# wangrui2025/GDKVM

Measured on AMD Instinct MI355X. Metric: frames/sec (GDKVM forward + argmax mask), EchoNet 112x112x32 clips, higher is better.
Workload: dtype bf16; 1 GPU; BASELINE.json configs[1]: EchoNet-Dynamic 112x112x32 bf16 inference, batch=16 per GPU; clips_per_gpu=16, frames_per_clip=32, image=112x112, heads=1, key_dim=64, rule=delta_sequential, world_size=1, ranks_seen=1

## Files before the change

gdkvm_amd/csrc/conv3x3_tile.hip:

```cpp
#include <atomic>
#include <type_traits>

#include "gdkvm_common.hpp"

namespace {

constexpr int CT_CK = 64;
constexpr int CT_PIX = 160;
constexpr int CT_SLOTS = CT_PIX / 16;
constexpr int CT_MAXMT = 13;
constexpr int CT_VARIANT_128 = 4, CT_VARIANT_64 = 3;

__device__ const uint4 g_ct_zero16 = {0, 0, 0, 0};

template <int I, int E, class F>
__device__ __forceinline__ void static_for_ct(F&& f)
{
    if constexpr (I < E) {
        f(std::integral_constant<int, I>{});
        static_for_ct<I + 1, E>(f);
    }
}

struct ConvTileArgs {
    const bf16_t* x; const bf16_t* w; const float* bias; const bf16_t* res; bf16_t* y;
    const bf16_t* x2; int C1;
    int N, H, W, C, K;
    int fpt, th, tiles_y, ntiles;
    int bw, bh, band_px, npieces;
    int relu;
    float inv_band, inv_bw, inv_tw, inv_w;
    int perm;
};

__device__ __forceinline__ int ct_div(int n, float inv) { return (int)(((float)n + 0.5f) * inv); }

__host__ __device__ __forceinline__ int ct_channel(int kt, int j, int perm)
{
    return perm ? 32 * (kt >> 1) + 8 * (j >> 2) + 4 * (kt & 1) + (j & 3) : 16 * kt + j;
}

template <int NWN, int NTW, bool PK, int NWV = 8, int MAXMT = CT_MAXMT>
__global__ __launch_bounds__(64 * NWV, (NWV == 4 ? 2 : 1)) void conv3x3_tile_kernel(ConvTileArgs a)
{
    constexpr int MW = NWV / NWN, MTW = (MAXMT + MW - 1) / MW;
    extern __shared__ __attribute__((aligned(16))) unsigned char ct_band[];
    const int tid = threadIdx.x, lane = tid & 63, li = lane & 15, g = lane >> 4;
    const int w = __builtin_amdgcn_readfirstlane(tid >> 6), wn = w % NWN, wm = w / NWN;
    const int H = a.H, W = a.W, C = a.C, K = a.K, BW = a.bw;
    const int band_bytes = a.npieces * 1024, nchunk = C / CT_CK;
    const int tpix = a.fpt * a.th * W;
    const int co0 = blockIdx.y * (16 * NTW * NWN) + 16 * NTW * wn;

    f32x4 bias4[NTW];
#pragma unroll
    for (int nt = 0; nt < NTW; ++nt) {
        const int kt = min(co0 / 16 + nt, K / 16 - 1);
        const float* bp = a.bias + ct_channel(kt, 4 * g, a.perm);
        asm volatile("global_load_dwordx4 %0, %1, off" : "=&v"(bias4[nt]) : "v"(bp) : "memory");
    }

    constexpr int PP = NWV == 8 ? 7 : 8;
    int g_pix[PP], g_meta[PP];
#pragma unroll
    for (int u = 0; u < PP; ++u) {
        const int j = w + NWV * u, d = 64 * j + lane, pix = d / CT_SLOTS, c = d - CT_SLOTS * pix;
        const int f = ct_div(pix, a.inv_band), r = pix - f * (a.bh * BW), by = ct_div(r, a.inv_bw), bx = r - by * BW;
        g_pix[u] = (f * H + by) * W + bx;
        const bool live = j < a.npieces && c < 8 && pix < a.band_px && bx >= 1 && bx <= W;
        g_meta[u] = live ? (by << 16 | (c * 8) << 8 | f) : -1;
    }
    struct Geo { const bf16_t* b1; const bf16_t* b2; int y0, nfr; };
    auto geo_of = [&](int tile) __attribute__((always_inline)) {
        const int ty = tile % a.tiles_y, fg = tile / a.tiles_y;
        Geo q;
        q.y0 = ty * a.th - 1;
        q.nfr = min(a.fpt, a.N - fg * a.fpt);
        const long long px0 = ((long long)fg * a.fpt * H + q.y0) * W - 1;
        q.b1 = a.x + px0 * (a.x2 ? a.C1 : C);
        q.b2 = a.x2 ? a.x2 + px0 * (C - a.C1) - a.C1 : a.x;
        return q;
    };
    auto fetch = [&](const Geo q, int chunk, int buf) __attribute__((always_inline)) {
        const int y0 = q.y0, nfr = q.nfr;
        const bool second = a.x2 != nullptr && chunk * CT_CK >= a.C1;
        const int cs = a.x2 ? (second ? C - a.C1 : a.C1) : C;
        const bf16_t* origin = (second ? q.b2 : q.b1) + chunk * CT_CK;
#pragma unroll
        for (int u = 0; u < PP; ++u) {
            const int j = w + NWV * u;
            const int yy = y0 + (g_meta[u] >> 16);
            const bool ok = g_meta[u] >= 0 && (unsigned)yy < (unsigned)H && (g_meta[u] & 255) < nfr;
            const bf16_t* src = ok ? origin + g_pix[u] * cs + ((g_meta[u] >> 8) & 255) : reinterpret_cast<const bf16_t*>(&g_ct_zero16);
            unsigned char* dst = j < a.npieces ? ct_band + buf * band_bytes + 1024 * j : ct_band + 2 * band_bytes;
            __builtin_amdgcn_global_load_lds(src, reinterpret_cast<__attribute__((address_space(3))) void*>(reinterpret_cast<uintptr_t>(dst)), 16, 0, 0);
        }
    };

    int tile = blockIdx.x;
    Geo cur = geo_of(min(tile, a.ntiles - 1));
    if (tile < a.ntiles) fetch(cur, 0, 0);

    unsigned pbase[MTW];
#pragma unroll
    for (int m = 0; m < MTW; ++m) {
        const int p = min(16 * (wm + MW * m) + li, tpix - 1);
        const int f = ct_div(p, a.inv_tw), r = p - f * (a.th * W), py = ct_div(r, a.inv_w), px = r - py * W;
        pbase[m] = (unsigned)(((f * a.bh + py) * BW + px) * CT_PIX + g * 16);
    }
    const bf16_t* wrow[NTW];
#pragma unroll
    for (int nt = 0; nt < NTW; ++nt) {
        const int kt = min(co0 / 16 + nt, K / 16 - 1);
        if constexpr (PK) wrow[nt] = a.w + (size_t)kt * (9 * C * 16) + lane * 8;
        else wrow[nt] = a.w + (size_t)ct_channel(kt, li, a.perm) * 9 * C + 8 * g;
    }

    const int nks = nchunk * 18;
    static_assert(NTW == 1 || NTW == 2, "wwait names the fragments of one or two output tiles");
    struct WF { bf16x8 f[NTW]; };
    auto wload = [&](WF& o, int ks) __attribute__((always_inline)) {
        ks = ks >= nks ? ks - nks : ks;
        size_t off;
        if constexpr (PK) off = (size_t)ks * 512;
        else {
            const int chunk = ks / 18, r = ks - 18 * chunk, tap = r >> 1, kh = r & 1;
            off = (size_t)tap * C + chunk * CT_CK + 32 * kh;
        }
#pragma unroll
        for (int nt = 0; nt < NTW; ++nt) asm volatile("global_load_dwordx4 %0, %1, off" : "=&v"(o.f[nt]) : "v"(wrow[nt] + off) : "memory");
    };
    auto wwait = [&](WF& o, auto nc) __attribute__((always_inline)) {
        constexpr int N = decltype(nc)::value;
        if constexpr (NTW == 1) asm volatile("s_waitcnt vmcnt(%1)" : "+v"(o.f[0]) : "n"(N) : "memory");
        else asm volatile("s_waitcnt vmcnt(%2)" : "+v"(o.f[0]), "+v"(o.f[1]) : "n"(N) : "memory");
    };
    int gc = 0;
    constexpr int WD = 3, KU = 6;
    WF wr[WD];
#pragma unroll
    for (int j = 0; j < WD; ++j) wload(wr[j], j);
    for (; tile < a.ntiles; tile += gridDim.x) {
        const Geo nxt = geo_of(min(tile + (int)gridDim.x, a.ntiles - 1));
        f32x4 acc[MTW][NTW];
#pragma unroll
        for (int m = 0; m < MTW; ++m)
#pragma unroll
            for (int nt = 0; nt < NTW; ++nt) acc[m][nt] = f32x4{0.f, 0.f, 0.f, 0.f};
        for (int chunk = 0; chunk < nchunk; ++chunk, ++gc) {
            const int buf = gc & 1;
            asm volatile("s_waitcnt vmcnt(%0) lgkmcnt(0)" ::"n"(WD * NTW) : "memory");
            asm volatile("s_barrier" ::: "memory");
            {
                const bool more = chunk + 1 < nchunk;
                Geo q;
                q.b1 = more ? cur.b1 : nxt.b1; q.b2 = more ? cur.b2 : nxt.b2; q.y0 = more ? cur.y0 : nxt.y0; q.nfr = more ? cur.nfr : nxt.nfr;
                fetch(q, more ? chunk + 1 : 0, buf ^ 1);
            }
            const unsigned char* band = ct_band + buf * band_bytes;
            auto load_x = [&](bf16x8 (&xb)[MTW], int r) __attribute__((always_inline)) {
                r = min(r, 17);
                const int tap = r >> 1, kh = r & 1, dy = tap / 3, dx = tap - 3 * dy;
                const unsigned off = (unsigned)((dy * BW + dx) * CT_PIX + kh * 64);
#pragma unroll
                for (int m = 0; m < MTW; ++m) {
                    xb[m] = *reinterpret_cast<const bf16x8*>(band + pbase[m] + off);
                }
            };
            auto mfmas = [&](const bf16x8 (&xb)[MTW], const WF& wfr) __attribute__((always_inline)) {
#pragma unroll
                for (int m = 0; m < MTW; ++m)
#pragma unroll
                    for (int nt = 0; nt < NTW; ++nt) {
                        acc[m][nt] = __builtin_amdgcn_mfma_f32_16x16x32_bf16(wfr.f[nt], xb[m], acc[m][nt], 0, 0, 0);
                    }
            };
            const int ksb = chunk * 18;
            bf16x8 xa[MTW], xb[MTW];
            load_x(xa, 0);
            auto trip = [&](int r0, auto firstc) __attribute__((always_inline)) {
                constexpr bool FIRST = decltype(firstc)::value;
                static_for_ct<0, KU>([&](auto jc) {
                    constexpr int j = decltype(jc)::value;
                    wwait(wr[j % WD], std::integral_constant<int, (WD - 1) * NTW + (FIRST && j < WD ? PP : 0)>{});
                    if constexpr (j % 2 == 0) { load_x(xb, r0 + j + 1); mfmas(xa, wr[j % WD]); }
                    else { load_x(xa, r0 + j + 1); mfmas(xb, wr[j % WD]); }
                    wload(wr[j % WD], ksb + r0 + j + WD);
                    __builtin_amdgcn_sched_barrier(0);
                });
            };
            trip(0, std::true_type{});
#pragma unroll 1
            for (int r0 = KU; r0 < 18; r0 += KU) trip(r0, std::false_type{});
        }
        {
            const int ty = tile % a.tiles_y, fg = tile / a.tiles_y;
            auto bf4 = [](uint2 rr) { return f32x4{__uint_as_float(rr.x << 16), __uint_as_float(rr.x & 0xffff0000u), __uint_as_float(rr.y << 16), __uint_as_float(rr.y & 0xffff0000u)}; };
            auto pk4 = [](const f32x4& v) { return make_uint2((unsigned)f32_to_bf16(v[0]) | ((unsigned)f32_to_bf16(v[1]) << 16), (unsigned)f32_to_bf16(v[2]) | ((unsigned)f32_to_bf16(v[3]) << 16)); };
            const float lo = a.relu ? 0.f : -INFINITY;
            typedef float f32x2 __attribute__((ext_vector_type(2)));
            if (NTW == 2 && a.perm) {
                if (co0 < K) {
                    unsigned o[MTW];
#pragma unroll
                    for (int m = 0; m < MTW; ++m) {
                        const int p = 16 * (wm + MW * m) + li;
                        const int pc = min(p, tpix - 1);
                        const int f = ct_div(pc, a.inv_tw), r = pc - f * (a.th * W), py = ct_div(r, a.inv_w), px = r - py * W;
                        const int n = fg * a.fpt + f, yy = ty * a.th + py;
                        o[m] = p < tpix && n < a.N && yy < H ? (unsigned)(((n * H + yy) * W + px) * K + co0 + 8 * g) : ~0u;
                    }
                    typedef unsigned u32x4 __attribute__((ext_vector_type(4)));
                    bf16_t* const yout = a.y;
                    const bf16_t* const resp = a.res;
                    const unsigned ofallback = (unsigned)(co0 + 8 * g);
                    auto finish = [&](auto resc) __attribute__((always_inline)) {
                        constexpr bool RES = decltype(resc)::value;
                        static_for_ct<0, (MTW + 3) / 4>([&](auto bc) {
                            constexpr int M0 = 4 * decltype(bc)::value, M1 = M0 + 4 < MTW ? M0 + 4 : MTW;
                            u32x4 rr[4] = {};
                            if constexpr (RES) {
#pragma unroll
                                for (int m = M0; m < M1; ++m)
                                {
                                    const bf16_t* const rp = resp + (o[m] != ~0u ? o[m] : ofallback);
                                    asm volatile("global_load_dwordx4 %0, %1, off" : "=&v"(rr[m - M0]) : "v"(rp) : "memory");
                                }
                                asm volatile("s_waitcnt vmcnt(0)" : "+v"(rr[0]), "+v"(rr[1]), "+v"(rr[2]), "+v"(rr[3]) :: "memory");
                            }
#pragma unroll
                            for (int m = M0; m < M1; ++m) {
                                f32x2 v[4];
#pragma unroll
                                for (int q = 0; q < 4; ++q)
                                    v[q] = f32x2{acc[m][q >> 1][2 * (q & 1)], acc[m][q >> 1][2 * (q & 1) + 1]} + f32x2{bias4[q >> 1][2 * (q & 1)], bias4[q >> 1][2 * (q & 1) + 1]};
                                if constexpr (RES) {
#pragma unroll
                                    for (int q = 0; q < 4; ++q) v[q] += f32x2{__uint_as_float(rr[m - M0][q] << 16), __uint_as_float(rr[m - M0][q] & 0xffff0000u)};
                                }
                                u32x4 ow;
#pragma unroll
                                for (int q = 0; q < 4; ++q) {
                                    v[q] = __builtin_elementwise_max(v[q], f32x2{lo, lo});
                                    ow[q] = (unsigned)f32_to_bf16(v[q][0]) | ((unsigned)f32_to_bf16(v[q][1]) << 16);
                                }
                                bf16_t* const yp = yout + o[m];
                                if (o[m] != ~0u) asm volatile("global_store_dwordx4 %0, %1, off\n\ts_nop 1" :: "v"(yp), "v"(ow) : "memory");
                            }
                        });
                    };
                    if (a.res) finish(std::true_type{}); else finish(std::false_type{});
                }
            } else {
#pragma unroll
                for (int m = 0; m < MTW; ++m) {
                    const int p = 16 * (wm + MW * m) + li;
                    if (p >= tpix) continue;
                    const int f = ct_div(p, a.inv_tw), r = p - f * (a.th * W), py = ct_div(r, a.inv_w), px = r - py * W;
                    const int n = fg * a.fpt + f, yy = ty * a.th + py;
                    if (n >= a.N || yy >= H) continue;
                    const size_t opix = (((size_t)n * H + yy) * W + px) * K;
#pragma unroll
                    for (int nt = 0; nt < NTW; ++nt) {
                        if (co0 + 16 * nt >= K) continue;
                        const size_t o = opix + ct_channel(co0 / 16 + nt, 4 * g, a.perm);
                        f32x4 v = acc[m][nt] + bias4[nt];
                        if (a.res) v += bf4(*reinterpret_cast<const uint2*>(a.res + o));
                        v = __builtin_elementwise_max(v, f32x4{lo, lo, lo, lo});
                        *reinterpret_cast<uint2*>(a.y + o) = pk4(v);
                    }
                }
            }
        }
        cur = nxt;
    }
    asm volatile("s_waitcnt vmcnt(0)" ::: "memory");
}

__global__ __launch_bounds__(256) void conv3x3_pack_kernel(const uint4* w, uint4* packed, int K, int C)
{
    const int nks = C / CT_CK * 18;
    const size_t total = (size_t)(K / 16) * nks * 64;
    for (size_t i = (size_t)blockIdx.x * 256 + threadIdx.x; i < total; i += (size_t)gridDim.x * 256) {
        const int lane = (int)(i & 63), li = lane & 15, g = lane >> 4;
        const size_t f = i >> 6;
        const int ks = (int)(f % nks), kt = (int)(f / nks);
        const int chunk = ks / 18, r = ks - 18 * chunk, tap = r >> 1, kh = r & 1;
        packed[i] = w[(((size_t)ct_channel(kt, li, K % 32 == 0) * 9 + tap) * C + chunk * CT_CK + 32 * kh + 8 * g) / 8];
    }
}

__global__ __launch_bounds__(256) void conv3x3_pack_dgrad_kernel(const bf16_t* w, uint4* packed, int K, int C)
{
    const int nks = K / CT_CK * 18;
    const size_t total = (size_t)(C / 16) * nks * 64;
    for (size_t i = (size_t)blockIdx.x * 256 + threadIdx.x; i < total; i += (size_t)gridDim.x * 256) {
        const int lane = (int)(i & 63), li = lane & 15, g = lane >> 4;
        const size_t f = i >> 6;
        const int ks = (int)(f % nks), ct = (int)(f / nks);
        const int chunk = ks / 18, r = ks - 18 * chunk, tap = r >> 1, kh = r & 1;
        const int c = ct_channel(ct, li, C % 32 == 0), ftap = 8 - tap;
        const bf16_t* src = w + ((size_t)(chunk * CT_CK + 32 * kh + 8 * g) * 9 + ftap) * C + c;
        unsigned short e[8];
#pragma unroll
        for (int j = 0; j < 8; ++j) e[j] = src[(size_t)j * 9 * C];
        packed[i] = make_uint4(e[0] | (unsigned)e[1] << 16, e[2] | (unsigned)e[3] << 16, e[4] | (unsigned)e[5] << 16, e[6] | (unsigned)e[7] << 16);
    }
}

}

struct PackTrainLayer { const float* w; uint4* fwd; uint4* dgrad; int K, C; long long sK, sC, sR, sS; };
struct PackTrainArgs { PackTrainLayer l[GDKVM_PACK_MAX_LAYERS]; };

namespace {
__global__ __launch_bounds__(256) void conv3x3_pack_train_kernel(PackTrainArgs a)
{
    const PackTrainLayer L = a.l[blockIdx.y];
    if (!L.w) return;
    const int K = L.K, C = L.C;
    const size_t nf = (size_t)(K / 16) * (C / CT_CK * 18) * 64, nd = (size_t)(C / 16) * (K / CT_CK * 18) * 64;
    auto bf = [](float x) { return (unsigned)f32_to_bf16(x); };
    for (size_t i = (size_t)blockIdx.x * 256 + threadIdx.x; i < nf + nd; i += (size_t)gridDim.x * 256) {
        const bool fwd = i < nf;
        const size_t ii = fwd ? i : i - nf;
        const int lane = (int)(ii & 63), li = lane & 15, g = lane >> 4;
        const size_t f = ii >> 6;
        float e[8];
        if (fwd) {
            const int nks = C / CT_CK * 18, ks = (int)(f % nks), kt = (int)(f / nks);
            const int chunk = ks / 18, r = ks - 18 * chunk, tap = r >> 1, kh = r & 1;
            const float* src = L.w + (long long)ct_channel(kt, li, K % 32 == 0) * L.sK + (long long)(tap / 3) * L.sR + (long long)(tap % 3) * L.sS
                               + (long long)(chunk * CT_CK + 32 * kh + 8 * g) * L.sC;
#pragma unroll
            for (int j = 0; j < 8; ++j) e[j] = src[(long long)j * L.sC];
        } else {
            const int nks = K / CT_CK * 18, ks = (int)(f % nks), ct = (int)(f / nks);
            const int chunk = ks / 18, r = ks - 18 * chunk, tap = r >> 1, kh = r & 1, ftap = 8 - tap;
            const float* src = L.w + (long long)ct_channel(ct, li, C % 32 == 0) * L.sC + (long long)(ftap / 3) * L.sR + (long long)(ftap % 3) * L.sS
                               + (long long)(chunk * CT_CK + 32 * kh + 8 * g) * L.sK;
#pragma unroll
            for (int j = 0; j < 8; ++j) e[j] = src[(long long)j * L.sK];
        }
        const uint4 o = make_uint4(bf(e[0]) | bf(e[1]) << 16, bf(e[2]) | bf(e[3]) << 16, bf(e[4]) | bf(e[5]) << 16, bf(e[6]) | bf(e[7]) << 16);
        (fwd ? L.fwd : L.dgrad)[ii] = o;
    }
}
}

extern "C" int gdkvm_conv3x3_pack_weights_train(int nlayers, const void* const* w, void* const* packed_fwd, void* const* packed_dgrad,
                                                const int* K, const int* C, const long long* strides, void* stream)
{
    if (nlayers < 0 || nlayers > GDKVM_PACK_MAX_LAYERS) return gdkvm_fail(GDKVM_ERR_SHAPE, "conv3x3_pack_weights_train: %d layers (at most %d per call)", nlayers, GDKVM_PACK_MAX_LAYERS);
    if (nlayers == 0) return GDKVM_OK;
    if (!w || !packed_fwd || !packed_dgrad || !K || !C || !strides) return gdkvm_fail(GDKVM_ERR_ARG, "conv3x3_pack_weights_train: null pointer");
    PackTrainArgs a{};
    for (int i = 0; i < nlayers; ++i) {
        if (K[i] <= 0 || C[i] <= 0 || K[i] % CT_CK || C[i] % CT_CK)
            return gdkvm_fail(GDKVM_ERR_SHAPE, "conv3x3_pack_weights_train: layer %d K=%d C=%d (multiples of 64)", i, K[i], C[i]);
        if (!w[i] || !packed_fwd[i] || !packed_dgrad[i] || !gdkvm_aligned16(packed_fwd[i]) || !gdkvm_aligned16(packed_dgrad[i]))
            return gdkvm_fail(GDKVM_ERR_ARG, "conv3x3_pack_weights_train: layer %d: null or unaligned pointer", i);
        a.l[i] = PackTrainLayer{static_cast<const float*>(w[i]), static_cast<uint4*>(packed_fwd[i]), static_cast<uint4*>(packed_dgrad[i]), K[i], C[i],
                                strides[4 * i], strides[4 * i + 1], strides[4 * i + 2], strides[4 * i + 3]};
    }
    if (int rc = gdkvm_check_device()) return rc;
    hipLaunchKernelGGL(conv3x3_pack_train_kernel, dim3(48, (unsigned)nlayers), dim3(256), 0, static_cast<hipStream_t>(stream), a);
    GDKVM_LAUNCH_CHECK("conv3x3_pack_train_kernel");
    return GDKVM_OK;
}

extern "C" int gdkvm_conv3x3_pack_weights_dgrad(const void* w, void* packed, int K, int C, int io_dtype, void* stream)
{
    if (io_dtype != GDKVM_BF16) return gdkvm_fail(GDKVM_ERR_DTYPE, "conv3x3_pack_weights_dgrad: only bf16 is implemented");
    if (K <= 0 || C <= 0 || K % CT_CK || C % 16) return gdkvm_fail(GDKVM_ERR_SHAPE, "conv3x3_pack_weights_dgrad: K=%d C=%d (K a multiple of 64, C of 16)", K, C);
    if (!w || !packed || !gdkvm_aligned16(w) || !gdkvm_aligned16(packed)) return gdkvm_fail(GDKVM_ERR_ARG, "conv3x3_pack_weights_dgrad: null or unaligned pointer");
    if (int rc = gdkvm_check_device()) return rc;
    const size_t total = (size_t)(C / 16) * (K / CT_CK * 18) * 64;
    hipLaunchKernelGGL(conv3x3_pack_dgrad_kernel, dim3((unsigned)((total + 255) / 256)), dim3(256), 0, static_cast<hipStream_t>(stream),
                       static_cast<const bf16_t*>(w), static_cast<uint4*>(packed), K, C);
    GDKVM_LAUNCH_CHECK("conv3x3_pack_dgrad_kernel");
    return GDKVM_OK;
}

extern "C" int gdkvm_conv3x3_pack_weights(const void* w, void* packed, int K, int C, int io_dtype, void* stream)
{
    if (io_dtype != GDKVM_BF16) return gdkvm_fail(GDKVM_ERR_DTYPE, "conv3x3_pack_weights: only bf16 is implemented");
    if (K <= 0 || C <= 0 || K % 16 || C % CT_CK) return gdkvm_fail(GDKVM_ERR_SHAPE, "conv3x3_pack_weights: K=%d C=%d (K a multiple of 16, C of 64)", K, C);
    if (!w || !packed || !gdkvm_aligned16(w) || !gdkvm_aligned16(packed)) return gdkvm_fail(GDKVM_ERR_ARG, "conv3x3_pack_weights: null or unaligned pointer");
    if (int rc = gdkvm_check_device()) return rc;
    const size_t total = (size_t)(K / 16) * (C / CT_CK * 18) * 64;
    hipLaunchKernelGGL(conv3x3_pack_kernel, dim3((unsigned)((total + 255) / 256)), dim3(256), 0, static_cast<hipStream_t>(stream),
                       static_cast<const uint4*>(w), static_cast<uint4*>(packed), K, C);
    GDKVM_LAUNCH_CHECK("conv3x3_pack_kernel");
    return GDKVM_OK;
}

namespace {
template <int NWN, int NTW, int NWV = 8, int MAXMT = CT_MAXMT>
void launch_tile(bool packed, dim3 grid, size_t lds, hipStream_t st, const ConvTileArgs& a)
{
    if (packed) hipLaunchKernelGGL((conv3x3_tile_kernel<NWN, NTW, true, NWV, MAXMT>), grid, dim3(64 * NWV), lds, st, a);
    else hipLaunchKernelGGL((conv3x3_tile_kernel<NWN, NTW, false, NWV, MAXMT>), grid, dim3(64 * NWV), lds, st, a);
}
template <int NWN, int NTW, int NWV = 8, int MAXMT = CT_MAXMT>
bool setattr_tile()
{
    return hipFuncSetAttribute(reinterpret_cast<const void*>(conv3x3_tile_kernel<NWN, NTW, true, NWV, MAXMT>), hipFuncAttributeMaxDynamicSharedMemorySize, 113 * 1024) == hipSuccess
        && hipFuncSetAttribute(reinterpret_cast<const void*>(conv3x3_tile_kernel<NWN, NTW, false, NWV, MAXMT>), hipFuncAttributeMaxDynamicSharedMemorySize, 113 * 1024) == hipSuccess;
}
}

int gdkvm_conv3x3_tile_launch(const void* x, const void* x2, int C1, const void* w, const float* bias, const void* residual, void* y,
                              int N, int C, int H, int W, int K, int relu, int variant, int packed, hipStream_t st)
{
    if (variant == 0 && K % 128 == 0 && CT_VARIANT_128 == 4) {
        if (gdkvm_conv3x3_tile_launch(x, x2, C1, w, bias, residual, y, N, C, H, W, K, relu, 4, packed, st) == 0) return 0;
        variant = 2;
    }
    if (variant == 0 && K % 128 != 0 && (H * W <= 16 * 7 || 2 * W <= 16 * 7)) {
        if (gdkvm_conv3x3_tile_launch(x, x2, C1, w, bias, residual, y, N, C, H, W, K, relu, 5, packed, st) == 0) return 0;
        variant = 3;
    }
    if (C % CT_CK || K % 16 || W > 64 || W < 1 || H < 1 || N < 1 || variant < 0 || variant > 5) return 1;
    if (variant == 4 && K % 128) return 1;
    const bool half = variant == 4 || variant == 5;
    if (x2 && (C1 <= 0 || C1 >= C || C1 % CT_CK)) return 1;
    ConvTileArgs a;
    a.x2 = static_cast<const bf16_t*>(x2); a.C1 = x2 ? C1 : C;
    a.x = static_cast<const bf16_t*>(x); a.w = static_cast<const bf16_t*>(w); a.bias = bias;
    a.res = static_cast<const bf16_t*>(residual); a.y = static_cast<bf16_t*>(y);
    a.N = N; a.H = H; a.W = W; a.C = C; a.K = K; a.relu = relu;
    const int maxpix = half ? 16 * 7 : 16 * CT_MAXMT;
    const int maxpieces = half ? 32 : 56;
    if (H * W <= maxpix) { a.th = H; a.fpt = maxpix / (H * W); a.tiles_y = 1; if (a.fpt > N) a.fpt = N; }
    else { a.fpt = 1; a.th = maxpix / W; if (a.th < 1) return 1; a.tiles_y = (H + a.th - 1) / a.th; }
    a.bw = W + 2; a.bh = a.th + 2;
    auto pieces = [&]() { a.band_px = a.fpt * a.bh * a.bw; return (a.band_px * CT_SLOTS + 63) / 64; };
    while (pieces() > maxpieces && a.fpt > 1) --a.fpt;
    while (pieces() > maxpieces && a.th > 1) { --a.th; a.bh = a.th + 2; a.tiles_y = (H + a.th - 1) / a.th; }
    a.npieces = pieces();
    if (a.npieces > maxpieces) return 1;
    a.inv_band = 1.0f / (float)(a.bh * a.bw); a.inv_bw = 1.0f / (float)a.bw;
    a.inv_tw = 1.0f / (float)(a.th * W); a.inv_w = 1.0f / (float)W;
    a.perm = K % 32 == 0;
    const long long groups = (N + a.fpt - 1) / a.fpt;
    const long long ntiles = groups * a.tiles_y;
    if (ntiles <= 0 || ntiles > 0x7fffffffLL) return 1;
    a.ntiles = (int)ntiles;
    if (variant == 0) variant = K % 128 == 0 ? 2 : CT_VARIANT_64;
    const int kwg = (variant == 2 || variant == 4) ? 128 : 64;
    const int gy = (K + kwg - 1) / kwg;
    const size_t lds = (size_t)2 * a.npieces * 1024 + 1024;
    int per = (half ? 512 : 256) / gy; if (per < 1) per = 1;
    const int gx = (int)(ntiles < per ? ntiles : per);
    static std::atomic<unsigned long long> done_mask{0};
    int dev = 0;
    if (hipGetDevice(&dev) != hipSuccess) return 1;
    const unsigned long long bit = 1ull << (dev & 63);
    if (!(done_mask.load(std::memory_order_relaxed) & bit)) {
        if (!setattr_tile<4, 1>() || !setattr_tile<4, 2>() || !setattr_tile<2, 2>() || !setattr_tile<4, 2, 4, 7>() || !setattr_tile<2, 2, 4, 7>()) return 1;
        done_mask.fetch_or(bit, std::memory_order_relaxed);
    }
    switch (variant) {
        case 1: launch_tile<4, 1>(packed, dim3(gx, gy), lds, st, a); break;
        case 2: launch_tile<4, 2>(packed, dim3(gx, gy), lds, st, a); break;
        case 4: launch_tile<4, 2, 4, 7>(packed, dim3(gx, gy), lds, st, a); break;
        case 5: launch_tile<2, 2, 4, 7>(packed, dim3(gx, gy), lds, st, a); break;
        default: launch_tile<2, 2>(packed, dim3(gx, gy), lds, st, a); break;
    }
    return 0;
}
```

gdkvm_amd/csrc/conv_dispatch.hip:

```cpp
#include "gdkvm_common.hpp"

int gdkvm_conv3x3_c64_launch(const void* x, const void* w, const float* bias, const void* residual, void* y, int N, int H, int W,
                             int relu, int packed, hipStream_t st);
int gdkvm_conv3x3_tile_launch(const void* x, const void* x2, int C1, const void* w, const float* bias, const void* residual, void* y,
                              int N, int C, int H, int W, int K, int relu, int variant, int packed, hipStream_t st);
int gdkvm_conv_igemm_launch(const void* x, const void* wpacked, const float* bias, const void* residual, void* y,
                            int N, int C, int H, int W, int K, int R, int S, int stride, int pad, int relu,
                            const void* w2packed, const float* bias2, void* y2, hipStream_t st);

extern "C" int gdkvm_conv_bias_act(const void* x, const void* w, const float* bias, const void* residual, void* y,
                                   int N, int C, int H, int W, int K, int R, int S, int stride, int pad, int relu, int kernel,
                                   int io_dtype, void* stream)
{
    if (io_dtype != GDKVM_BF16) return gdkvm_fail(GDKVM_ERR_DTYPE, "conv_bias_act: only bf16 is implemented");
    if (N < 0 || C <= 0 || H <= 0 || W <= 0 || K <= 0 || R <= 0 || S <= 0 || stride <= 0 || pad < 0 || C % 8 || K % 8
        || H + 2 * pad < R || W + 2 * pad < S)
        return gdkvm_fail(GDKVM_ERR_SHAPE, "conv_bias_act: N=%d C=%d H=%d W=%d K=%d %dx%d stride %d pad %d (C, K multiples of 8)",
                          N, C, H, W, K, R, S, stride, pad);
    const bool packed = kernel & GDKVM_CONV_PACKED_WEIGHTS;
    kernel &= ~GDKVM_CONV_PACKED_WEIGHTS;
    if (kernel != 0 && (kernel < 4 || kernel > 11)) return gdkvm_fail(GDKVM_ERR_ARG, "conv_bias_act: kernel=%d (0 = by shape, 4, 5, 6..8, 9, 10, 11)", kernel);
    if (kernel == 9) {
        if (!packed) return gdkvm_fail(GDKVM_ERR_ARG, "conv_bias_act: kernel 9 reads the gdkvm_conv_igemm_pack_weights copy of the weights (flag %d)", GDKVM_CONV_PACKED_WEIGHTS);
        if (C % 32 || K % 128) return gdkvm_fail(GDKVM_ERR_SHAPE, "conv_bias_act: kernel 9 needs C a multiple of 32 and K of 128 (C=%d K=%d)", C, K);
        if (N == 0) return GDKVM_OK;
        if (!x || !w || !bias || !y) return gdkvm_fail(GDKVM_ERR_ARG, "conv_bias_act: null pointer");
        if (!gdkvm_aligned16(x) || !gdkvm_aligned16(w) || !gdkvm_aligned16(y) || !gdkvm_aligned16(bias) || (residual && !gdkvm_aligned16(residual)))
            return gdkvm_fail(GDKVM_ERR_ARG, "conv_bias_act: pointers must be 16-byte aligned");
        if (int rc = gdkvm_check_device()) return rc;
        if (gdkvm_conv_igemm_launch(x, w, bias, residual, y, N, C, H, W, K, R, S, stride, pad, relu, nullptr, nullptr, nullptr, static_cast<hipStream_t>(stream)))
            return gdkvm_fail(GDKVM_ERR_SHAPE, "conv_bias_act: N=%d C=%d H=%d W=%d K=%d %dx%d stride %d pad %d is too large for 32-bit offsets", N, C, H, W, K, R, S, stride, pad);
        GDKVM_LAUNCH_CHECK("conv_igemm_kernel");
        return GDKVM_OK;
    }
    if (packed && (C % 64 || K % 16))
        return gdkvm_fail(GDKVM_ERR_ARG, "conv_bias_act: packed weights need C a multiple of 64 and K of 16 (C=%d K=%d)", C, K);
    if (!(R == 3 && S == 3 && stride == 1 && pad == 1))
        return gdkvm_fail(GDKVM_ERR_SHAPE, "conv_bias_act: %dx%d stride %d pad %d is not served by the 3x3 / 1 / 1 kernels: kernel 9 (the "
                                           "implicit-GEMM kernel, packed weights) or the framework convolution + gdkvm_bias_act", R, S, stride, pad);
    if (N == 0) return GDKVM_OK;
    if (!x || !w || !bias || !y) return gdkvm_fail(GDKVM_ERR_ARG, "conv_bias_act: null pointer");
    if (!gdkvm_aligned16(x) || !gdkvm_aligned16(w) || !gdkvm_aligned16(y) || !gdkvm_aligned16(bias) || (residual && !gdkvm_aligned16(residual)))
        return gdkvm_fail(GDKVM_ERR_ARG, "conv_bias_act: pointers must be 16-byte aligned");
    if ((size_t)N * H * W * C >= (1ull << 31) || (size_t)N * H * W * K >= (1ull << 31))
        return gdkvm_fail(GDKVM_ERR_SHAPE, "conv_bias_act: tensor too large for 32-bit offsets");
    if (int rc = gdkvm_check_device()) return rc;
    hipStream_t st = static_cast<hipStream_t>(stream);
    const bool c64 = C == 64 && K == 64;
    if (kernel == 4 && !c64) return gdkvm_fail(GDKVM_ERR_SHAPE, "conv_bias_act: kernel 4 serves 64 -> 64 channels only (C=%d K=%d)", C, K);
    if (kernel == 4 || (kernel == 0 && c64)) {
        if (gdkvm_conv3x3_c64_launch(x, w, bias, residual, y, N, H, W, relu, packed ? 1 : 0, st)) return gdkvm_fail(GDKVM_ERR_SHAPE, "conv_bias_act: too many tiles");
        GDKVM_LAUNCH_CHECK("conv3x3_c64_kernel");
        return GDKVM_OK;
    }
    if (gdkvm_conv3x3_tile_launch(x, nullptr, 0, w, bias, residual, y, N, C, H, W, K, relu, kernel >= 10 ? kernel - 6 : (kernel >= 6 ? kernel - 5 : 0), packed ? 1 : 0, st))
        return gdkvm_fail(GDKVM_ERR_SHAPE, "conv_bias_act: C=%d K=%d %dx%d is not served by the hand-written kernels (C a multiple of 64, K of "
                                           "16, rows of at most 64 pixels): use the framework convolution + gdkvm_bias_act", C, K, H, W);
    GDKVM_LAUNCH_CHECK("conv3x3_tile_kernel");
    return GDKVM_OK;
}

extern "C" int gdkvm_conv_cat_bias_act(const void* x1, const void* x2, const void* w, const float* bias, const void* residual, void* y,
                                       int N, int C1, int C2, int H, int W, int K, int relu, int kernel, int io_dtype, void* stream)
{
    if (io_dtype != GDKVM_BF16) return gdkvm_fail(GDKVM_ERR_DTYPE, "conv_cat_bias_act: only bf16 is implemented");
    const bool packed = kernel & GDKVM_CONV_PACKED_WEIGHTS;
    kernel &= ~GDKVM_CONV_PACKED_WEIGHTS;
    if (kernel != 0 && (kernel < 5 || kernel > 11 || kernel == 9)) return gdkvm_fail(GDKVM_ERR_ARG, "conv_cat_bias_act: kernel=%d (0, 5..8, 10, 11)", kernel);
    if (N < 0 || C1 <= 0 || C2 <= 0 || C1 % 64 || C2 % 64 || H <= 0 || W <= 0 || K <= 0 || K % 16)
        return gdkvm_fail(GDKVM_ERR_SHAPE, "conv_cat_bias_act: N=%d C1=%d C2=%d H=%d W=%d K=%d (C1, C2 multiples of 64, K of 16)", N, C1, C2, H, W, K);
    if (N == 0) return GDKVM_OK;
    if (!x1 || !x2 || !w || !bias || !y) return gdkvm_fail(GDKVM_ERR_ARG, "conv_cat_bias_act: null pointer");
    if (!gdkvm_aligned16(x1) || !gdkvm_aligned16(x2) || !gdkvm_aligned16(w) || !gdkvm_aligned16(y) || !gdkvm_aligned16(bias) || (residual && !gdkvm_aligned16(residual)))
        return gdkvm_fail(GDKVM_ERR_ARG, "conv_cat_bias_act: pointers must be 16-byte aligned");
    if ((size_t)N * H * W * (C1 + C2) >= (1ull << 31) || (size_t)N * H * W * K >= (1ull << 31))
        return gdkvm_fail(GDKVM_ERR_SHAPE, "conv_cat_bias_act: tensor too large for 32-bit offsets");
    if (int rc = gdkvm_check_device()) return rc;
    if (gdkvm_conv3x3_tile_launch(x1, x2, C1, w, bias, residual, y, N, C1 + C2, H, W, K, relu, kernel >= 10 ? kernel - 6 : (kernel >= 6 ? kernel - 5 : 0), packed ? 1 : 0,
                                  static_cast<hipStream_t>(stream)))
        return gdkvm_fail(GDKVM_ERR_SHAPE, "conv_cat_bias_act: %dx%d is not served (rows of at most 64 pixels)", H, W);
    GDKVM_LAUNCH_CHECK("conv3x3_tile_kernel");
    return GDKVM_OK;
}

extern "C" int gdkvm_conv_down_bias_act(const void* x, const void* w, const float* bias, void* y, int relu,
                                        const void* w_down, const float* bias_down, void* y_down,
                                        int N, int C, int H, int W, int K, int R, int S, int stride, int pad, int io_dtype, void* stream)
{
    if (io_dtype != GDKVM_BF16) return gdkvm_fail(GDKVM_ERR_DTYPE, "conv_down_bias_act: only bf16 is implemented");
    if (N < 0 || C <= 0 || H <= 0 || W <= 0 || K <= 0 || R <= 0 || S != R || !(R & 1) || stride <= 0 || pad != R / 2 || C % 32 || K % 128)
        return gdkvm_fail(GDKVM_ERR_SHAPE, "conv_down_bias_act: N=%d C=%d H=%d W=%d K=%d %dx%d stride %d pad %d (odd square window, pad = R/2, "
                                           "C a multiple of 32, K of 128)", N, C, H, W, K, R, S, stride, pad);
    if (N == 0) return GDKVM_OK;
    if (!x || !w || !bias || !y || !w_down || !y_down) return gdkvm_fail(GDKVM_ERR_ARG, "conv_down_bias_act: null pointer");
    const void* ptrs[] = {x, w, bias, y, w_down, y_down};
    for (const void* p : ptrs) if (!gdkvm_aligned16(p)) return gdkvm_fail(GDKVM_ERR_ARG, "conv_down_bias_act: pointers must be 16-byte aligned");
    if (bias_down && !gdkvm_aligned16(bias_down)) return gdkvm_fail(GDKVM_ERR_ARG, "conv_down_bias_act: pointers must be 16-byte aligned");
    if (int rc = gdkvm_check_device()) return rc;
    if (gdkvm_conv_igemm_launch(x, w, bias, nullptr, y, N, C, H, W, K, R, S, stride, pad, relu, w_down, bias_down, y_down, static_cast<hipStream_t>(stream)))
        return gdkvm_fail(GDKVM_ERR_SHAPE, "conv_down_bias_act: tensor too large for 32-bit offsets");
    GDKVM_LAUNCH_CHECK("conv_igemm_kernel");
    return GDKVM_OK;
}
```

gdkvm_amd/csrc/epilogue.hip:

```cpp
#include <type_traits>

#include <stdlib.h>
#include "gdkvm_common.hpp"

namespace {

template <int IO, bool FIXED>
__global__ __launch_bounds__(256) void bias_act_kernel(const void* x, const float* bias, const void* res, void* y,
                                                       size_t nvec, int C, int relu)
{
    constexpr int V = IO == GDKVM_F32 ? 4 : 8;
    constexpr int UNR = 4;
    typedef uint4 vec_t;
    const vec_t* xv = static_cast<const vec_t*>(x);
    const vec_t* rv = static_cast<const vec_t*>(res);
    vec_t* yv = static_cast<vec_t*>(y);
    const size_t stride = (size_t)gridDim.x * 256;
    float bfix[V];
    if constexpr (FIXED) {
        const int c0 = (int)((((size_t)blockIdx.x * 256 + threadIdx.x) * V) % (size_t)C);
#pragma unroll
        for (int j = 0; j < V; j += 4) {
            const f32x4 b4 = *reinterpret_cast<const f32x4*>(bias + c0 + j);
            bfix[j] = b4[0]; bfix[j + 1] = b4[1]; bfix[j + 2] = b4[2]; bfix[j + 3] = b4[3];
// ... 71 lines not shown
        uint4 win[9];
#pragma unroll
        for (int dy = 0; dy < 3; ++dy)
#pragma unroll
            for (int dx = 0; dx < 3; ++dx) {
                const int ih = 2 * oh - 1 + dy, iw = 2 * ow - 1 + dx;
                const bool ok = ih >= 0 && ih < H && iw >= 0 && iw < W;
                const int hh = ok ? ih : 2 * oh, ww = ok ? iw : 2 * ow;
                win[3 * dy + dx] = xv[(((size_t)n * Hp + hh) * Wp + ww) * cg + c];
            }
        float m[V];
#pragma unroll
        for (int j = 0; j < V; ++j) m[j] = -INFINITY;
#pragma unroll
        for (int t = 0; t < 9; ++t) {
            const unsigned w4[4] = {win[t].x, win[t].y, win[t].z, win[t].w};
#pragma unroll
            for (int j = 0; j < 4; ++j) {
                if constexpr (IO == GDKVM_F32) m[j] = fmaxf(m[j], __uint_as_float(w4[j]));
                else {
                    m[2 * j] = fmaxf(m[2 * j], __uint_as_float(w4[j] << 16));
                    m[2 * j + 1] = fmaxf(m[2 * j + 1], __uint_as_float(w4[j] & 0xffff0000u));
                }
            }
        }
#pragma unroll
        for (int j = 0; j < V; j += 4) {
            const f32x4 b4 = *reinterpret_cast<const f32x4*>(bias + c * V + j);
#pragma unroll
            for (int q = 0; q < 4; ++q) m[j + q] = fmaxf(m[j + q] + b4[q], 0.f);
        }
        uint4 o;
        if constexpr (IO == GDKVM_F32) {
            o.x = __float_as_uint(m[0]); o.y = __float_as_uint(m[1]); o.z = __float_as_uint(m[2]); o.w = __float_as_uint(m[3]);
        } else {
            o.x = (unsigned)f32_to_bf16(m[0]) | ((unsigned)f32_to_bf16(m[1]) << 16);
            o.y = (unsigned)f32_to_bf16(m[2]) | ((unsigned)f32_to_bf16(m[3]) << 16);
            o.z = (unsigned)f32_to_bf16(m[4]) | ((unsigned)f32_to_bf16(m[5]) << 16);
            o.w = (unsigned)f32_to_bf16(m[6]) | ((unsigned)f32_to_bf16(m[7]) << 16);
        }
        yv[i] = o;
    }
}

template <int IO>
__global__ __launch_bounds__(256) void stem_s2d_kernel(const void* x, void* out, int N, int C, int H, int W, int Cp)
{
    typedef typename std::conditional<IO == GDKVM_F32, float, bf16_t>::type T;
    const T* xi = static_cast<const T*>(x);
    T* o = static_cast<T*>(out);
    const int Ho = H / 2, Wo = W / 2;
    const size_t total = (size_t)N * Ho * Wo;
    for (size_t i = (size_t)blockIdx.x * 256 + threadIdx.x; i < total; i += (size_t)gridDim.x * 256) {
        const int j = (int)(i % Wo);
        const size_t r = i / Wo;
        const int ih = (int)(r % Ho), n = (int)(r / Ho);
        T* dst = o + i * Cp;
        if constexpr (IO == GDKVM_BF16) {
            if (Cp == 16 && C <= 4) {
                unsigned pr[8] = {0, 0, 0, 0, 0, 0, 0, 0};
                for (int c = 0; c < C; ++c) {
                    const bf16_t* src = xi + (((size_t)n * C + c) * H + 2 * ih) * W + 2 * j;
                    pr[2 * c] = *reinterpret_cast<const unsigned*>(src);
                    pr[2 * c + 1] = *reinterpret_cast<const unsigned*>(src + W);
                }
                reinterpret_cast<uint4*>(dst)[0] = make_uint4(pr[0], pr[1], pr[2], pr[3]);
                reinterpret_cast<uint4*>(dst)[1] = make_uint4(pr[4], pr[5], pr[6], pr[7]);
                continue;
            }
        }
        for (int c = 0; c < C; ++c) {
            const T* src = xi + (((size_t)n * C + c) * H + 2 * ih) * W + 2 * j;
            dst[4 * c + 0] = src[0]; dst[4 * c + 1] = src[1]; dst[4 * c + 2] = src[W]; dst[4 * c + 3] = src[W + 1];
        }
        for (int c = 4 * C; c < Cp; ++c) dst[c] = T(0);
    }
}

}

extern "C" int gdkvm_bias_act(const void* x, const float* bias, const void* residual, void* y,
                              size_t rows, int C, int relu, int io_dtype, void* stream)
{
    if (C <= 0) return gdkvm_fail(GDKVM_ERR_SHAPE, "bias_act: C=%d", C);
    if (io_dtype != GDKVM_F32 && io_dtype != GDKVM_BF16) return gdkvm_fail(GDKVM_ERR_DTYPE, "bias_act: io_dtype=%d", io_dtype);
    const int V = io_dtype == GDKVM_F32 ? 4 : 8;
    if (C % V) return gdkvm_fail(GDKVM_ERR_SHAPE, "bias_act: C=%d must be a multiple of %d", C, V);
    if (rows == 0) return GDKVM_OK;
    if (!x || !bias || !y) return gdkvm_fail(GDKVM_ERR_ARG, "bias_act: null pointer");
    if (!gdkvm_aligned16(x) || !gdkvm_aligned16(y) || !gdkvm_aligned16(bias) || (residual && !gdkvm_aligned16(residual)))
        return gdkvm_fail(GDKVM_ERR_ARG, "bias_act: pointers must be 16-byte aligned");
    if (int rc = gdkvm_check_device()) return rc;
    const size_t nvec = rows * (size_t)C / V;
    size_t blocks = (nvec + 255) / 256;
    if (blocks > 256 * 8) blocks = 256 * 8;
    hipStream_t st = static_cast<hipStream_t>(stream);
    const bool fixed = (blocks * 256) % (size_t)(C / V) == 0;
#define GDKVM_BA(IO, FX) hipLaunchKernelGGL((bias_act_kernel<IO, FX>), dim3((unsigned)blocks), dim3(256), 0, st, x, bias, residual, y, nvec, C, relu)
    if (io_dtype == GDKVM_F32) { if (fixed) GDKVM_BA(GDKVM_F32, true); else GDKVM_BA(GDKVM_F32, false); }
    else { if (fixed) GDKVM_BA(GDKVM_BF16, true); else GDKVM_BA(GDKVM_BF16, false); }
#undef GDKVM_BA
    GDKVM_LAUNCH_CHECK("bias_act_kernel");
    return GDKVM_OK;
}

namespace {

__device__ __forceinline__ void unpack8(const uint4& a, float (&v)[8])
{
    const unsigned w[4] = {a.x, a.y, a.z, a.w};
#pragma unroll
    for (int j = 0; j < 4; ++j) { v[2 * j] = __uint_as_float(w[j] << 16); v[2 * j + 1] = __uint_as_float(w[j] & 0xffff0000u); }
}

__global__ __launch_bounds__(256) void upsample_cat_bf16_kernel(const bf16_t* lo, const bf16_t* skip, bf16_t* out,
                                                                int Nimg, int hl, int wl, int H, int W, int C1, int C2,
                                                                float sy, float sx, float inv_c1n, float inv_c2n, float inv_h)
{
    auto qdiv = [](int n, float inv) { return (int)(((float)n + 0.5f) * inv); };
    const int C = C1 + C2, c1n = C1 / 8, c2n = C2 / 8, n1 = W * c1n, n2 = W * c2n, tid = threadIdx.x;
    constexpr int MAXV = 2;
    const bool exact2x = H == 2 * hl && W == 2 * wl;
    for (int row = blockIdx.x; row < Nimg * H; row += gridDim.x) {
        const int n = qdiv(row, inv_h), y = row - n * H;
        const float fy = fmaxf(sy * ((float)y + 0.5f) - 0.5f, 0.f);
        const int y0 = (int)fy, y1 = min(y0 + 1, hl - 1);
        const float ly = fy - (float)y0, hy = 1.f - ly;
        const bf16_t* lo0 = lo + ((size_t)n * hl + y0) * wl * C1;
        const bf16_t* lo1 = lo + ((size_t)n * hl + y1) * wl * C1;
        const bf16_t* sk = skip + (size_t)row * W * C2;
        bf16_t* orow = out + (size_t)row * W * C;
        uint4 cp[MAXV];
#pragma unroll
        for (int u = 0; u < MAXV; ++u) cp[u] = n2 ? *reinterpret_cast<const uint4*>(sk + min(u * 256 + tid, n2 - 1) * 8) : make_uint4(0u, 0u, 0u, 0u);
        if (exact2x) {
            const int nu = (wl + 1) * c1n;
            for (int u0 = 0; u0 < nu; u0 += 256) {
                const int u = min(u0 + tid, nu - 1);
                const int jq = qdiv(u, inv_c1n), c = (u - jq * c1n) * 8, jp = jq - 1;
                const int x0 = max(jp, 0), x1 = min(jp + 1, wl - 1);
                const uint4 t00 = *reinterpret_cast<const uint4*>(lo0 + x0 * C1 + c), t01 = *reinterpret_cast<const uint4*>(lo0 + x1 * C1 + c);
                const uint4 t10 = *reinterpret_cast<const uint4*>(lo1 + x0 * C1 + c), t11 = *reinterpret_cast<const uint4*>(lo1 + x1 * C1 + c);
                if (u0 + tid >= nu) continue;
                float a[8], b[8], cc[8], d[8];
                unpack8(t00, a); unpack8(t01, b); unpack8(t10, cc); unpack8(t11, d);
#pragma unroll
                for (int e = 0; e < 2; ++e) {
                    const int x = 2 * jp + 1 + e;
                    if (x < 0 || x >= W) continue;
                    const float lx = e ? 0.75f : 0.25f, hx = 1.f - lx;
                    unsigned r[4];
#pragma unroll
                    for (int q = 0; q < 4; ++q) {
                        const float v0 = hy * (hx * a[2 * q] + lx * b[2 * q]) + ly * (hx * cc[2 * q] + lx * d[2 * q]);
                        const float v1 = hy * (hx * a[2 * q + 1] + lx * b[2 * q + 1]) + ly * (hx * cc[2 * q + 1] + lx * d[2 * q + 1]);
                        r[q] = (unsigned)f32_to_bf16(v0) | ((unsigned)f32_to_bf16(v1) << 16);
                    }
                    *reinterpret_cast<uint4*>(orow + x * C + c) = make_uint4(r[0], r[1], r[2], r[3]);
                }
            }
        } else
        for (int j0 = 0; j0 < n1; j0 += MAXV * 256) {
            uint4 t[MAXV][4];
            float lx[MAXV];
            int oidx[MAXV];
#pragma unroll
            for (int u = 0; u < MAXV; ++u) {
                const int j = min(j0 + u * 256 + tid, n1 - 1);
                const int x = qdiv(j, inv_c1n), c = (j - x * c1n) * 8;
                const float fx = fmaxf(sx * ((float)x + 0.5f) - 0.5f, 0.f);
                const int x0 = (int)fx, x1 = min(x0 + 1, wl - 1);
                lx[u] = fx - (float)x0;
                oidx[u] = x * C + c;
                t[u][0] = *reinterpret_cast<const uint4*>(lo0 + x0 * C1 + c);
                t[u][1] = *reinterpret_cast<const uint4*>(lo0 + x1 * C1 + c);
                t[u][2] = *reinterpret_cast<const uint4*>(lo1 + x0 * C1 + c);
                t[u][3] = *reinterpret_cast<const uint4*>(lo1 + x1 * C1 + c);
            }
#pragma unroll
            for (int u = 0; u < MAXV; ++u) {
                if (j0 + u * 256 + tid >= n1) continue;
                const float hx = 1.f - lx[u];
                float a[8], b[8], cc[8], d[8];
                unpack8(t[u][0], a); unpack8(t[u][1], b); unpack8(t[u][2], cc); unpack8(t[u][3], d);
                unsigned r[4];
#pragma unroll
                for (int q = 0; q < 4; ++q) {
                    const float v0 = hy * (hx * a[2 * q] + lx[u] * b[2 * q]) + ly * (hx * cc[2 * q] + lx[u] * d[2 * q]);
                    const float v1 = hy * (hx * a[2 * q + 1] + lx[u] * b[2 * q + 1]) + ly * (hx * cc[2 * q + 1] + lx[u] * d[2 * q + 1]);
                    r[q] = (unsigned)f32_to_bf16(v0) | ((unsigned)f32_to_bf16(v1) << 16);
                }
                *reinterpret_cast<uint4*>(orow + oidx[u]) = make_uint4(r[0], r[1], r[2], r[3]);
            }
        }
#pragma unroll
        for (int u = 0; u < MAXV; ++u) {
            const int jc = u * 256 + tid;
            if (jc < n2) {
                const int x = qdiv(jc, inv_c2n);
                *reinterpret_cast<uint4*>(orow + x * C + C1 + (jc - x * c2n) * 8) = cp[u];
            }
        }
        for (int jc = MAXV * 256 + tid; jc < n2; jc += 256) {
            const int x = qdiv(jc, inv_c2n);
            *reinterpret_cast<uint4*>(orow + x * C + C1 + (jc - x * c2n) * 8) = *reinterpret_cast<const uint4*>(sk + jc * 8);
        }
    }
}

__global__ __launch_bounds__(256) void upsample_cat_bf16_2x_kernel(const bf16_t* lo, const bf16_t* skip, bf16_t* out,
                                                                   int Nimg, int hl, int wl, int C1, int C2, float inv_c1n, float inv_c2n, float inv_hp)
{
    auto qdiv = [](int n, float inv) { return (int)(((float)n + 0.5f) * inv); };
    const int H = 2 * hl, W = 2 * wl, C = C1 + C2, c1n = C1 / 8, c2n = C2 / 8, n2 = W * c2n, tid = threadIdx.x;
    const int nu = (wl + 1) * c1n, hp = hl + 1;
    for (int rp = blockIdx.x; rp < Nimg * hp; rp += gridDim.x) {
        const int n = qdiv(rp, inv_hp), ip = rp - n * hp - 1;
        const int r0 = max(ip, 0), r1 = min(ip + 1, hl - 1);
        const bf16_t* lo0 = lo + ((size_t)n * hl + r0) * wl * C1;
        const bf16_t* lo1 = lo + ((size_t)n * hl + r1) * wl * C1;
        constexpr int MAXV = 2;
        uint4 cp[2][MAXV];
#pragma unroll
        for (int ey = 0; ey < 2; ++ey) {
            const int y = min(max(2 * ip + 1 + ey, 0), H - 1);
            const bf16_t* sk = skip + ((size_t)n * H + y) * W * C2;
#pragma unroll
            for (int u = 0; u < MAXV; ++u) cp[ey][u] = n2 ? *reinterpret_cast<const uint4*>(sk + min(u * 256 + tid, n2 - 1) * 8) : make_uint4(0u, 0u, 0u, 0u);
        }
        for (int u0 = 0; u0 < nu; u0 += 256) {
            const int u = min(u0 + tid, nu - 1);
            const int jq = qdiv(u, inv_c1n), c = (u - jq * c1n) * 8, jp = jq - 1;
            const int x0 = max(jp, 0), x1 = min(jp + 1, wl - 1);
            const uint4 t00 = *reinterpret_cast<const uint4*>(lo0 + x0 * C1 + c), t01 = *reinterpret_cast<const uint4*>(lo0 + x1 * C1 + c);
            const uint4 t10 = *reinterpret_cast<const uint4*>(lo1 + x0 * C1 + c), t11 = *reinterpret_cast<const uint4*>(lo1 + x1 * C1 + c);
            if (u0 + tid >= nu) continue;
            float a[8], b[8], cc[8], d[8];
            unpack8(t00, a); unpack8(t01, b); unpack8(t10, cc); unpack8(t11, d);
#pragma unroll
            for (int ey = 0; ey < 2; ++ey) {
                const int y = 2 * ip + 1 + ey;
                if (y < 0 || y >= H) continue;
                const float fy = fmaxf(0.5f * ((float)y + 0.5f) - 0.5f, 0.f);
                const float ly = fy - (float)(int)fy, hy = 1.f - ly;
                bf16_t* orow = out + ((size_t)n * H + y) * W * C;
#pragma unroll
                for (int e = 0; e < 2; ++e) {
                    const int x = 2 * jp + 1 + e;
                    if (x < 0 || x >= W) continue;
                    const float lx = e ? 0.75f : 0.25f, hx = 1.f - lx;
                    unsigned r[4];
#pragma unroll
                    for (int q = 0; q < 4; ++q) {
                        const float v0 = hy * (hx * a[2 * q] + lx * b[2 * q]) + ly * (hx * cc[2 * q] + lx * d[2 * q]);
                        const float v1 = hy * (hx * a[2 * q + 1] + lx * b[2 * q + 1]) + ly * (hx * cc[2 * q + 1] + lx * d[2 * q + 1]);
                        r[q] = (unsigned)f32_to_bf16(v0) | ((unsigned)f32_to_bf16(v1) << 16);
                    }
                    *reinterpret_cast<uint4*>(orow + x * C + c) = make_uint4(r[0], r[1], r[2], r[3]);
                }
            }
        }
#pragma unroll
        for (int ey = 0; ey < 2; ++ey) {
            const int y = 2 * ip + 1 + ey;
            if (y < 0 || y >= H) continue;
            bf16_t* orow = out + ((size_t)n * H + y) * W * C;
            const bf16_t* sk = skip + ((size_t)n * H + y) * W * C2;
#pragma unroll
            for (int u = 0; u < MAXV; ++u) {
                const int jc = u * 256 + tid;
                if (jc < n2) {
                    const int x = qdiv(jc, inv_c2n);
                    *reinterpret_cast<uint4*>(orow + x * C + C1 + (jc - x * c2n) * 8) = cp[ey][u];
                }
            }
            for (int jc = MAXV * 256 + tid; jc < n2; jc += 256) {
                const int x = qdiv(jc, inv_c2n);
                *reinterpret_cast<uint4*>(orow + x * C + C1 + (jc - x * c2n) * 8) = *reinterpret_cast<const uint4*>(sk + jc * 8);
            }
        }
    }
}

template <int IO>
__global__ __launch_bounds__(256) void maxpool_fwd_kernel(const void* x, void* y, unsigned char* idx,
                                                          int N, int H, int W, int C, int Ho, int Wo)
{
    constexpr int V = IO == GDKVM_F32 ? 4 : 8;
    const int cg = C / V;
    const size_t total = (size_t)N * Ho * Wo * cg;
    const uint4* xv = static_cast<const uint4*>(x);
    uint4* yv = static_cast<uint4*>(y);
    for (size_t i = (size_t)blockIdx.x * 256 + threadIdx.x; i < total; i += (size_t)gridDim.x * 256) {
        const int c = (int)(i % cg);
        size_t p = i / cg;
        const int ow = (int)(p % Wo); p /= Wo;
        const int oh = (int)(p % Ho);
        const int n = (int)(p / Ho);
        uint4 win[9];
        bool ok[9];
#pragma unroll
        for (int dy = 0; dy < 3; ++dy)
#pragma unroll
            for (int dx = 0; dx < 3; ++dx) {
                const int ih = 2 * oh - 1 + dy, iw = 2 * ow - 1 + dx;
                ok[3 * dy + dx] = ih >= 0 && ih < H && iw >= 0 && iw < W;
                const int hh = ok[3 * dy + dx] ? ih : 2 * oh, ww = ok[3 * dy + dx] ? iw : 2 * ow;
                win[3 * dy + dx] = xv[(((size_t)n * H + hh) * W + ww) * cg + c];
            }
        float m[V];
        unsigned char best[V];
#pragma unroll
        for (int j = 0; j < V; ++j) { m[j] = -INFINITY; best[j] = 4; }
        bool first = true;
#pragma unroll
        for (int t = 0; t < 9; ++t) {
            if (!ok[t]) continue;
            const unsigned w4[4] = {win[t].x, win[t].y, win[t].z, win[t].w};
            float v[V];
#pragma unroll
            for (int j = 0; j < 4; ++j) {
                if constexpr (IO == GDKVM_F32) v[j] = __uint_as_float(w4[j]);
                else { v[2 * j] = __uint_as_float(w4[j] << 16); v[2 * j + 1] = __uint_as_float(w4[j] & 0xffff0000u); }
            }
#pragma unroll
            for (int j = 0; j < V; ++j)
                if (first || v[j] > m[j] || v[j] != v[j]) { m[j] = v[j]; best[j] = (unsigned char)t; }
            first = false;
        }
        uint4 o;
        if constexpr (IO == GDKVM_F32) {
            o.x = __float_as_uint(m[0]); o.y = __float_as_uint(m[1]); o.z = __float_as_uint(m[2]); o.w = __float_as_uint(m[3]);
            *reinterpret_cast<unsigned*>(idx + i * 4) = best[0] | (best[1] << 8) | (best[2] << 16) | ((unsigned)best[3] << 24);
        } else {
            o.x = (__float_as_uint(m[0]) >> 16) | (__float_as_uint(m[1]) & 0xffff0000u);
            o.y = (__float_as_uint(m[2]) >> 16) | (__float_as_uint(m[3]) & 0xffff0000u);
            o.z = (__float_as_uint(m[4]) >> 16) | (__float_as_uint(m[5]) & 0xffff0000u);
            o.w = (__float_as_uint(m[6]) >> 16) | (__float_as_uint(m[7]) & 0xffff0000u);
            uint2 b;
            b.x = best[0] | (best[1] << 8) | (best[2] << 16) | ((unsigned)best[3] << 24);
            b.y = best[4] | (best[5] << 8) | (best[6] << 16) | ((unsigned)best[7] << 24);
            *reinterpret_cast<uint2*>(idx + i * 8) = b;
        }
        yv[i] = o;
    }
}

template <int IO>
__global__ __launch_bounds__(256) void maxpool_bwd_kernel(const void* dy, const unsigned char* idx, void* dx,
                                                          int N, int H, int W, int C, int Ho, int Wo)
{
    constexpr int V = IO == GDKVM_F32 ? 4 : 8;
    const int cg = C / V;
    const size_t total = (size_t)N * H * W * cg;
    const uint4* dv = static_cast<const uint4*>(dy);
    uint4* xv = static_cast<uint4*>(dx);
    for (size_t i = (size_t)blockIdx.x * 256 + threadIdx.x; i < total; i += (size_t)gridDim.x * 256) {
        const int c = (int)(i % cg);
        size_t p = i / cg;
        const int iw = (int)(p % W); p /= W;
        const int ih = (int)(p % H);
        const int n = (int)(p / H);
        const int oh0 = ih >> 1, ow0 = iw >> 1;
        uint4 g[4];
        unsigned bt[4][2];
        int tap[4];
#pragma unroll
        for (int a = 0; a < 2; ++a)
#pragma unroll
            for (int b = 0; b < 2; ++b) {
                const int oh = oh0 + a, ow = ow0 + b;
                const bool ok = (a == 0 || ((ih & 1) && oh < Ho)) && (b == 0 || ((iw & 1) && ow < Wo)) && oh < Ho && ow < Wo;
                const size_t o = (((size_t)n * Ho + (ok ? oh : oh0 < Ho ? oh0 : Ho - 1)) * Wo + (ok ? ow : ow0 < Wo ? ow0 : Wo - 1)) * cg + c;
                g[2 * a + b] = dv[o];
                if constexpr (IO == GDKVM_F32) { bt[2 * a + b][0] = *reinterpret_cast<const unsigned*>(idx + o * 4); bt[2 * a + b][1] = 0; }
                else { const uint2 t = *reinterpret_cast<const uint2*>(idx + o * 8); bt[2 * a + b][0] = t.x; bt[2 * a + b][1] = t.y; }
                tap[2 * a + b] = ok ? 3 * (ih - (2 * oh - 1)) + (iw - (2 * ow - 1)) : 255;
            }
        float acc[V];
#pragma unroll
        for (int j = 0; j < V; ++j) acc[j] = 0.f;
#pragma unroll
        for (int q = 0; q < 4; ++q) {
            const unsigned w4[4] = {g[q].x, g[q].y, g[q].z, g[q].w};
#pragma unroll
            for (int j = 0; j < V; ++j) {
                const unsigned wt = (bt[q][j >> 2] >> (8 * (j & 3))) & 0xffu;
                float d;
                if constexpr (IO == GDKVM_F32) d = __uint_as_float(w4[j]);
                else d = (j & 1) ? __uint_as_float(w4[j >> 1] & 0xffff0000u) : __uint_as_float(w4[j >> 1] << 16);
                acc[j] += (int)wt == tap[q] ? d : 0.f;
            }
        }
        uint4 o;
        if constexpr (IO == GDKVM_F32) {
            o.x = __float_as_uint(acc[0]); o.y = __float_as_uint(acc[1]); o.z = __float_as_uint(acc[2]); o.w = __float_as_uint(acc[3]);
        } else {
            o.x = (unsigned)f32_to_bf16(acc[0]) | ((unsigned)f32_to_bf16(acc[1]) << 16);
            o.y = (unsigned)f32_to_bf16(acc[2]) | ((unsigned)f32_to_bf16(acc[3]) << 16);
            o.z = (unsigned)f32_to_bf16(acc[4]) | ((unsigned)f32_to_bf16(acc[5]) << 16);
            o.w = (unsigned)f32_to_bf16(acc[6]) | ((unsigned)f32_to_bf16(acc[7]) << 16);
        }
        xv[i] = o;
    }
}

__device__ __forceinline__ float tap_weight(int o, int i, float s, int n_in)
{
// ... 228 lines not shown
```

gdkvm_amd/csrc/gdkvm_common.hpp:

```cpp
#pragma once
#include <hip/hip_runtime.h>
#include <stdint.h>

#include "gdkvm.h"

typedef float f32x4 __attribute__((ext_vector_type(4)));
typedef unsigned short bf16_t;
typedef __bf16 bf16x8 __attribute__((ext_vector_type(8)));

#define GDKVM_DK 64
#define GDKVM_MAX_N 4096
#define GDKVM_EPS_NORM 1e-12f

int gdkvm_fail(int code, const char* fmt, ...);
int gdkvm_check_device(void);
int gdkvm_zero_async(void* p, size_t bytes, hipStream_t st);
static inline bool gdkvm_aligned16(const void* p) { return (reinterpret_cast<uintptr_t>(p) & 15u) == 0; }

#define GDKVM_LAUNCH_CHECK(name)                                                        \
    do {                                                                                \
        hipError_t e__ = hipGetLastError();                                             \
        if (e__ != hipSuccess) return gdkvm_fail(GDKVM_ERR_LAUNCH, "%s: %s", name, hipGetErrorString(e__)); \
    } while (0)

__host__ __device__ static inline size_t gdkvm_conv_s2_dgrad_pack_elems(int Cf, int Kf, int cls, int with_down)
{
    const int taps = (1 + (cls >> 1)) * (1 + (cls & 1)) + (cls == 0 && with_down ? 1 : 0);
    return (size_t)taps * Kf * Cf;
}

__device__ __forceinline__ float bf16_to_f32(bf16_t u) { return __uint_as_float(((unsigned)u) << 16); }
__device__ __forceinline__ bf16_t f32_to_bf16(float f)
{
    return __builtin_bit_cast(unsigned short, static_cast<__bf16>(f));
}
__device__ __forceinline__ float sigmoidf_(float x) { return 1.0f / (1.0f + __expf(-x)); }

template <int IO>
__device__ __forceinline__ f32x4 load4(const void* base, size_t off)
{
    if constexpr (IO == GDKVM_F32) {
        return *reinterpret_cast<const f32x4*>(static_cast<const float*>(base) + off);
    } else {
        const uint2 u = *reinterpret_cast<const uint2*>(static_cast<const bf16_t*>(base) + off);
        f32x4 r;
        r[0] = __uint_as_float(u.x << 16); r[1] = __uint_as_float(u.x & 0xffff0000u);
        r[2] = __uint_as_float(u.y << 16); r[3] = __uint_as_float(u.y & 0xffff0000u);
        return r;
    }
}
template <int IO>
__device__ __forceinline__ float load1(const void* base, size_t off)
{
    if constexpr (IO == GDKVM_F32) return static_cast<const float*>(base)[off];
    else return bf16_to_f32(static_cast<const bf16_t*>(base)[off]);
}
template <int IO>
__device__ __forceinline__ void store1(void* base, size_t off, float x)
{
    if constexpr (IO == GDKVM_F32) static_cast<float*>(base)[off] = x;
    else static_cast<bf16_t*>(base)[off] = f32_to_bf16(x);
}

__device__ __forceinline__ f32x4 mfma4(float a, float b, f32x4 c)
{
    return __builtin_amdgcn_mfma_f32_16x16x4f32(a, b, c, 0, 0, 0);
}
```

gdkvm_amd/model.py:

```python
from __future__ import annotations

from dataclasses import dataclass
import os
from typing import NamedTuple, Optional, Tuple

import torch
import torch.nn as nn
import torch.nn.functional as F

from . import ops

_RULES = {"gated_linear": ops.RULE_GATED_LINEAR, "delta_parallel": ops.RULE_DELTA_PARALLEL,
          "delta_sequential": ops.RULE_DELTA_SEQUENTIAL}

_KEY_REMAP: dict = {}


@dataclass
class GDKVMConfig:
    in_channels: int = 3
    num_classes: int = 2
    heads: int = 1
    key_dim: int = 64
    value_dim: int = 256
# ... 81 lines not shown
    if _STRICT:
        raise RuntimeError(msg + " [GDKVM_STRICT=1]")
    if (layer, why) not in _FALLBACKS_SEEN:
        _FALLBACKS_SEEN.add((layer, why))
        import warnings
        warnings.warn(msg, RuntimeWarning, stacklevel=3)


def _describe(conv: nn.Conv2d, x: torch.Tensor) -> str:
    return (f"Conv2d({conv.in_channels}->{conv.out_channels}, k={tuple(conv.kernel_size)}, s={tuple(conv.stride)}) on "
            f"{tuple(x.shape)} {str(x.dtype).replace('torch.', '')}")


_BN_COUNTED_BY_MODEL = [False]
_FEEDBACK_PASS = [False]
_CLIP_PIPELINE = True


def _bn_act(bn: nn.BatchNorm2d, x: torch.Tensor, relu: bool, residual: Optional[torch.Tensor] = None) -> torch.Tensor:
    v = 8 if x.dtype == torch.bfloat16 else 4
    track = bn.track_running_stats and not _FEEDBACK_PASS[0]
    if (x.is_cuda and bn.training and bn.affine and x.dtype in (torch.bfloat16, torch.float32) and bn.weight.dtype == torch.float32
            and x.shape[1] % v == 0 and x.shape[1] // v <= 256):
        momentum = bn.momentum
        if track:
            if not _BN_COUNTED_BY_MODEL[0]:
                bn.num_batches_tracked.add_(1)
            if momentum is None:
                momentum = 1.0 / float(bn.num_batches_tracked)
        res = None if residual is None else residual.to(x.dtype)
        return ops.bn_act(x, bn.weight, bn.bias, bn.running_mean if track else None,
                          bn.running_var if track else None, res, momentum or 0.0, bn.eps, relu)
    if _FEEDBACK_PASS[0] and bn.training:
        y = F.batch_norm(x, None, None, bn.weight, bn.bias, True, 0.0, bn.eps)
    else:
        if _BN_COUNTED_BY_MODEL[0] and bn.training and bn.track_running_stats:
            bn.num_batches_tracked.sub_(1)
        y = bn(x)
    if residual is not None:
        y = y + residual
    return F.relu(y, inplace=True) if relu else y


def _conv(conv: nn.Conv2d, x: torch.Tensor) -> torch.Tensor:
    train = torch.is_grad_enabled() or _FEEDBACK_PASS[0]
    if (train and isinstance(conv, nn.Conv2d) and conv.bias is None and conv.padding_mode == "zeros"
            and ops.conv3x3_train_served(x, conv.weight, conv.stride, conv.padding, conv.dilation, conv.groups)):
        return ops.conv3x3(x, conv.weight)
    if train:
        _library_fallback(x, _describe(conv, x), "training build: only stride-1 3x3 layers with channel counts in multiples of 64, "
                          "the stem and the strided blocks of the default widths are hand-written")
    return conv(x)


class BasicBlock(nn.Module):
    def __init__(self, cin, cout, stride):
        super().__init__()
        self.conv1 = nn.Conv2d(cin, cout, 3, stride, 1, bias=False)
        self.bn1 = _bn(cout)
        self.conv2 = nn.Conv2d(cout, cout, 3, 1, 1, bias=False)
        self.bn2 = _bn(cout)
        self.down = None
        if stride != 1 or cin != cout:
            self.down = nn.Sequential(nn.Conv2d(cin, cout, 1, stride, bias=False), _bn(cout))

    def forward(self, x):
        if isinstance(self.conv1, FusedConv):
            pair = self.conv1.with_down(x, self.down) if self.down is not None else None
            if pair is not None:
                return self.conv2(pair[0], pair[1])
            skip = x if self.down is None else self.down(x)
            return self.conv2(self.conv1(x), skip.contiguous(memory_format=torch.channels_last) if skip.is_cuda else skip)
        if (self.down is None and torch.is_grad_enabled() and x.requires_grad and self.conv1.bias is None
                and self.conv1.padding_mode == "zeros"
                and ops.conv3x3_train_served(x, self.conv1.weight, self.conv1.stride, self.conv1.padding, self.conv1.dilation, self.conv1.groups)):
            y1, xs = ops.conv3x3_fork(x, self.conv1.weight)
            y = _bn_act(self.bn1, y1, True)
            return _bn_act(self.bn2, _conv(self.conv2, y), True, xs)
        if (self.down is not None and torch.is_grad_enabled() and isinstance(self.conv1, nn.Conv2d)
                and isinstance(self.down[0], nn.Conv2d) and ops.conv_s2_block_served(x, self.conv1, self.down[0])):
            y1, yd = ops.conv_s2_block(x, self.conv1.weight, self.down[0].weight)
            y = _bn_act(self.bn1, y1, True)
            return _bn_act(self.bn2, _conv(self.conv2, y), True, _bn_act(self.down[1], yd, False))
        y = _bn_act(self.bn1, _conv(self.conv1, x), True)
        skip = x if self.down is None else _bn_act(self.down[1], self.down[0](x), False)
        return _bn_act(self.bn2, _conv(self.conv2, y), True, skip)


class Encoder(nn.Module):

    def __init__(self, cin, widths):
        super().__init__()
        w4, w8, w16 = widths
        self.stem = nn.Sequential(nn.Conv2d(cin, w4, 7, 2, 3, bias=False), _bn(w4), nn.ReLU(inplace=True),
                                  nn.MaxPool2d(3, 2, 1))
        self.layer1 = nn.Sequential(BasicBlock(w4, w4, 1), BasicBlock(w4, w4, 1))
        self.layer2 = nn.Sequential(BasicBlock(w4, w8, 2), BasicBlock(w8, w8, 1))
        self.layer3 = nn.Sequential(BasicBlock(w8, w16, 2), BasicBlock(w16, w16, 1))

    def forward(self, x):
        s = self.stem
        if len(s) == 4 and isinstance(s[1], nn.BatchNorm2d):
            if torch.is_grad_enabled() and isinstance(s[0], nn.Conv2d) and ops.stem_conv_served(x, s[0]):
                x = ops.stem_conv(x, s[0].weight)
            else:
                if torch.is_grad_enabled():
                    _library_fallback(x, "encoder.stem: " + _describe(s[0], x), "training stem kernel serves 7x7 / stride 2 / <= 4 input channels / 64 outputs in bf16")
                x = s[0](x)
            p, bn = s[3], s[1]
            pool_ok = isinstance(p, nn.MaxPool2d) and (p.kernel_size, p.stride, p.padding, p.dilation, p.ceil_mode) == (3, 2, 1, 1, False)
            if (pool_ok and bn.training and bn.affine and bn.weight.dtype == torch.float32 and ops.bn_relu_pool_served(x)):
                momentum = bn.momentum
                if bn.track_running_stats:
                    if not _BN_COUNTED_BY_MODEL[0]:
                        bn.num_batches_tracked.add_(1)
                    if momentum is None:
                        momentum = 1.0 / float(bn.num_batches_tracked)
                x = ops.bn_relu_pool(x, bn.weight, bn.bias, bn.running_mean if bn.track_running_stats else None,
                                     bn.running_var if bn.track_running_stats else None, momentum or 0.0, bn.eps)
                f4 = self.layer1(x)
                f8 = self.layer2(f4)
                return f4, f8, self.layer3(f8)
            x = _bn_act(bn, x, True)
            if (x.is_cuda and isinstance(p, nn.MaxPool2d) and (p.kernel_size, p.stride, p.padding, p.dilation, p.ceil_mode) == (3, 2, 1, 1, False)
                    and x.shape[1] % (8 if x.dtype == torch.bfloat16 else 4) == 0 and x.dtype in (torch.bfloat16, torch.float32)):
                x = ops.maxpool3x3s2(x)
            else:
                x = p(x)
        else:
            x = s(x)
        f4 = self.layer1(x)
        f8 = self.layer2(f4)
        return f4, f8, self.layer3(f8)


def _rows_aligned16(x: torch.Tensor) -> torch.Tensor:
    row = x[0].numel() * x.element_size()
    if row % 16 == 0 and x.data_ptr() % 16 == 0 and x.is_contiguous():
        return x
    per = 16 // x.element_size()
    n = x[0].numel()
    padded = (n + per - 1) // per * per
    buf = torch.empty((x.shape[0], padded), dtype=x.dtype, device=x.device)
    buf[:, :n].copy_(x.reshape(x.shape[0], n))
    return buf[:, :n].unflatten(1, x.shape[1:]) if x.dim() > 2 else buf[:, :n]


class UpBlock(nn.Module):
    def __init__(self, cin, cskip, cout):
        super().__init__()
        self.conv = nn.Sequential(nn.Conv2d(cin + cskip, cout, 3, 1, 1, bias=False), _bn(cout), nn.ReLU(inplace=True),
                                  nn.Conv2d(cout, cout, 3, 1, 1, bias=False), _bn(cout), nn.ReLU(inplace=True))

    def forward(self, x, skip):
        c = self.conv
        if (isinstance(c[0], FusedConv) and not torch.is_grad_enabled() and x.is_cuda and x.dtype == torch.bfloat16
                and skip.dtype == torch.bfloat16 and c[0].cat_served(x.shape[1], skip.shape[1], skip.shape[-1])):
            u = ops.upsample_bilinear(x.contiguous(memory_format=torch.channels_last), skip.shape[2:])
            y = c[0].forward_cat(u, skip)
            for m in list(c)[1:]:
                y = m(y)
            return y
        if (x.is_cuda and x.dtype == torch.bfloat16 and skip.dtype == torch.bfloat16
                and x.shape[1] % 8 == 0 and skip.shape[1] % 8 == 0):
            x = ops.upsample_cat(x.contiguous(memory_format=torch.channels_last),
                                 skip.contiguous(memory_format=torch.channels_last))
        else:
            x = torch.cat([F.interpolate(x, size=skip.shape[-2:], mode="bilinear", align_corners=False), skip], 1)
        if len(c) == 6 and isinstance(c[1], nn.BatchNorm2d):
            return _bn_act(c[4], _conv(c[3], _bn_act(c[1], _conv(c[0], x), True)), True)
        return c(x)


class HeadFeature(NamedTuple):
    feature: torch.Tensor
    weight: torch.Tensor
    bias: torch.Tensor


class Decoder(nn.Module):
    def __init__(self, cp, widths, ncls):
        super().__init__()
        w4, w8, _ = widths
        self.up8 = UpBlock(cp, w8, w8)
        self.up4 = UpBlock(w8, w4, w4)
        self.head = nn.Conv2d(w4, ncls, 1)

    def forward(self, f, f8, f4, size, head_fused=False):
        y = self.up4(self.up8(f, f8), f4)
        hd = self.head
        v = 8 if y.dtype == torch.bfloat16 else 4
        g = y.shape[1] // v
        if (y.is_cuda and not torch.is_grad_enabled() and y.dtype in (torch.bfloat16, torch.float32) and hd.kernel_size == (1, 1)
                and hd.stride == (1, 1) and hd.padding == (0, 0) and hd.groups == 1 and hd.bias is not None and y.shape[1] % v == 0
                and g <= 64 and g & (g - 1) == 0 and hd.out_channels <= g and y.is_contiguous(memory_format=torch.channels_last)):
            w32, b32 = _packs_of(self).get(self, (hd.weight, hd.bias), (y.device,), lambda: (
                hd.weight.detach().reshape(hd.out_channels, -1).float().contiguous(), hd.bias.detach().float().contiguous()))
            if head_fused and size is None:
                return HeadFeature(y, w32, b32)
            x = ops.head_logits(y, w32, b32)
        elif torch.is_grad_enabled() and ops.head_served(y, hd):
            x = ops.head(y, hd.weight, hd.bias)
        else:
            _library_fallback(y, "decoder.head: " + _describe(hd, y), "head kernels serve a 1x1 convolution with bias on a channels_last bf16 / fp32 feature of 8 ... 512 channels")
            x = hd(y)
        return x if size is None else F.interpolate(x, size=size, mode="bilinear", align_corners=False)


def _fold_bn(conv: nn.Conv2d, bn: nn.BatchNorm2d) -> nn.Conv2d:
    fused = nn.Conv2d(conv.in_channels, conv.out_channels, conv.kernel_size, conv.stride, conv.padding,
                      conv.dilation, conv.groups, bias=True).to(conv.weight.device, conv.weight.dtype)
    scale = bn.weight / torch.sqrt(bn.running_var + bn.eps)
    fused.weight.data = conv.weight * scale.reshape(-1, 1, 1, 1)
    b0 = conv.bias if conv.bias is not None else torch.zeros_like(bn.running_mean)
    fused.bias.data = bn.bias + (b0 - bn.running_mean) * scale
    return fused


class FusedConv(nn.Module):

    def __init__(self, conv: nn.Conv2d, relu: bool):
        super().__init__()
        self.conv = nn.Conv2d(conv.in_channels, conv.out_channels, conv.kernel_size, conv.stride, conv.padding,
                              conv.dilation, conv.groups, bias=False).to(conv.weight.device, conv.weight.dtype)
        self.conv.weight.data = conv.weight.data
        self.epi = _EpilogueBias(conv.bias.data.float() if conv.bias is not None else torch.zeros(conv.out_channels, device=conv.weight.device))
        self.relu = relu

    @staticmethod
    def _tile(cin: int, cout: int, stride: int, has_res: bool, width: int = 0) -> Optional[int]:
        if stride != 1 or cin % 64 or cout % 16:
            return None
        if cin == 64 and cout == 64:
            return 4
        return 5 if width <= 64 else None

    def _packed(self, device, igemm: bool = False):
        pack = ops.conv_igemm_pack_weights if igemm else ops.conv3x3_pack_weights
        return _packs_of(self).get(self, (self.conv.weight,), (device, igemm), lambda: pack(self.conv.weight))

    def with_down(self, x, down):
        cv = self.conv
        d = down[0] if isinstance(down, nn.Sequential) and len(down) == 1 else None
        if not (isinstance(d, FusedConv) and getattr(d, "bias_folded_downstream", False) and not d.relu
                and not getattr(self, "bias_folded_downstream", False) and x.is_cuda and x.dtype == torch.bfloat16
                and cv.kernel_size == (3, 3) and cv.padding == (1, 1) and cv.dilation == (1, 1) and cv.groups == 1
                and cv.stride[0] == cv.stride[1] and d.conv.kernel_size == (1, 1) and d.conv.stride == cv.stride
                and d.conv.padding == (0, 0) and d.conv.groups == 1 and d.conv.in_channels == cv.in_channels
                and d.conv.out_channels == cv.out_channels and cv.in_channels % 32 == 0 and cv.out_channels % 128 == 0
                and cv.weight.dtype == torch.bfloat16 and d.conv.weight.dtype == torch.bfloat16
                and cv.weight.is_contiguous(memory_format=torch.channels_last)
                and self._tile(cv.in_channels, cv.out_channels, cv.stride[0], False, x.shape[-1]) is None):
            return None
        dw = d.conv.weight if d.conv.weight.is_contiguous(memory_format=torch.channels_last) else d.conv.weight.contiguous(memory_format=torch.channels_last)
        return ops.conv_down_bias_act(x.contiguous(memory_format=torch.channels_last), cv.weight, self.epi.bias, self._packed(x.device, igemm=True),
                                      dw, d._packed(x.device, igemm=True), None, cv.stride[0], self.relu)

    def cat_served(self, c1: int, c2: int, width: int) -> bool:
        cv = self.conv
        return (not getattr(self, "bias_folded_downstream", False) and cv.kernel_size == (3, 3) and cv.groups == 1
                and cv.dilation == (1, 1) and cv.stride == (1, 1) and cv.padding == (1, 1) and cv.weight.is_cuda
                and cv.weight.dtype == torch.bfloat16 and cv.weight.is_contiguous(memory_format=torch.channels_last)
                and c1 % 64 == 0 and c2 % 64 == 0 and c1 + c2 == cv.in_channels and cv.out_channels % 16 == 0 and width <= 64)

    def forward_cat(self, x1, x2):
        cl = torch.channels_last
        return ops.conv_cat_bias_act(x1.contiguous(memory_format=cl), x2.contiguous(memory_format=cl), self.conv.weight, self.epi.bias,
                                     None, self.relu, 0, self._packed(x1.device))

    def forward(self, x, residual=None):
        cv = self.conv
        folded = getattr(self, "bias_folded_downstream", False)
        if (not folded and x.is_cuda and x.dtype == torch.bfloat16 and cv.kernel_size == (3, 3) and cv.groups == 1
                and cv.dilation == (1, 1) and cv.stride[0] == cv.stride[1] and cv.padding == (1, 1) and cv.weight.dtype == torch.bfloat16
                and cv.in_channels % 8 == 0 and cv.out_channels % 8 == 0 and cv.weight.is_contiguous(memory_format=torch.channels_last)):
            tile = self._tile(cv.in_channels, cv.out_channels, cv.stride[0], residual is not None, x.shape[-1])
            if tile is not None:
                packed = self._packed(x.device) if tile in (4, 5) else None
                return ops.conv_bias_act(x.contiguous(memory_format=torch.channels_last), cv.weight, self.epi.bias, residual,
                                         cv.stride[0], 1, self.relu, tile, packed)
            if cv.in_channels % 32 == 0 and cv.out_channels % 128 == 0:
                return ops.conv_bias_act(x.contiguous(memory_format=torch.channels_last), cv.weight, self.epi.bias, residual,
                                         cv.stride[0], 1, self.relu, ops.CONV_KERNEL_IGEMM, self._packed(x.device, igemm=True))
        _library_fallback(x, _describe(cv, x), "inference build: the hand-written kernels take bf16 channels_last 3x3 / pad 1 layers with channel counts "
                          "in multiples of 8 (strided: 32 in, 128 out) and the 1x1 branch fused into a strided block")
        y = self.conv(x)
        if folded:
            return y
        if not y.is_cuda:
            y = y + self.epi.bias.to(y.dtype).reshape(1, -1, 1, 1)
            y = y if residual is None else y + residual
            return F.relu(y) if self.relu else y
        y = y.contiguous(memory_format=torch.channels_last)
        return ops.bias_act_(y, self.epi.bias, residual, self.relu)


class FusedConvPool(FusedConv):

    S2D_CH = 16

    def enable_s2d(self):
        cv = self.conv
        if (cv.kernel_size, cv.stride, cv.padding, cv.dilation, cv.groups) != ((7, 7), (2, 2), (3, 3), (1, 1), 1) \
                or 4 * cv.in_channels > self.S2D_CH:
            return self
        w7 = cv.weight.data
        w4 = torch.zeros(cv.out_channels, self.S2D_CH, 4, 4, dtype=w7.dtype, device=w7.device)
        for a in range(-2, 2):
            for p_ in range(2):
                u = 2 * a + p_ + 3
                if not 0 <= u <= 6:
                    continue
                for b in range(-2, 2):
                    for q_ in range(2):
                        v = 2 * b + q_ + 3
                        if 0 <= v <= 6:
                            w4[:, p_ * 2 + q_:4 * cv.in_channels:4, a + 2, b + 2] = w7[:, :, u, v]
        self.register_buffer("w_s2d", w4.contiguous(memory_format=torch.channels_last))
        return self

    def forward(self, x, residual=None):
        if x.is_cuda and getattr(self, "w_s2d", None) is not None and x.shape[2] % 2 == 0 and x.shape[3] % 2 == 0:
            if (x.dtype == torch.bfloat16 and x.shape[1] <= 4 and self.w_s2d.dtype == torch.bfloat16
                    and tuple(self.w_s2d.shape) == (64, 16, 4, 4) and self.w_s2d.is_contiguous(memory_format=torch.channels_last)):
                return ops.stem_conv_pool_nchw(x.contiguous(), self.w_s2d, self.epi.bias)
            xs = ops.stem_s2d(x.contiguous(), self.S2D_CH)
            y = F.conv2d(xs, self.w_s2d, None, 1, 2)
            return ops.bias_relu_maxpool(y.contiguous(memory_format=torch.channels_last)[:, :, :x.shape[2] // 2, :x.shape[3] // 2],
                                         self.epi.bias)
        _library_fallback(x, "encoder.stem: " + _describe(self.conv, x), "inference stem kernel serves 7x7 / stride 2 / pad 3, <= 4 input channels, 64 outputs, bf16, even sizes")
        y = self.conv(x)
        if not y.is_cuda:
            return F.max_pool2d(F.relu(y + self.epi.bias.to(y.dtype).reshape(1, -1, 1, 1)), 3, 2, 1)
        return ops.bias_relu_maxpool(y.contiguous(memory_format=torch.channels_last), self.epi.bias)


class _EpilogueBias(nn.Module):

    def __init__(self, bias):
        super().__init__()
        self.bias = nn.Parameter(bias, requires_grad=False)

    def _apply(self, fn, recurse=True):
        def keep_fp32(t):
            r = fn(t)
            return r.float() if r.is_floating_point() else r
        return super()._apply(keep_fp32, recurse)


def _fold_sequential(seq: nn.Sequential) -> nn.Sequential:
    mods, out, i = list(seq), [], 0
    while i < len(mods):
        if isinstance(mods[i], nn.Conv2d) and i + 1 < len(mods) and isinstance(mods[i + 1], nn.BatchNorm2d):
            out.append(_fold_bn(mods[i], mods[i + 1])); i += 2
        else:
            out.append(mods[i]); i += 1
    return nn.Sequential(*out)


class KPFFParams(nn.Module):

    def _apply(self, fn, recurse=True):
        def keep_fp32(t):
            r = fn(t)
            return r.float() if r.is_floating_point() else r
        return super()._apply(keep_fp32, recurse)

    def __init__(self, ck, cv, cp):
        super().__init__()
        cin = cp + ck + cv
        self.wa = nn.Parameter(torch.empty(2 * cp, cin))
        self.ba = nn.Parameter(torch.zeros(2 * cp))
        self.wl = nn.Parameter(torch.empty(cp, ck))
        self.wg = nn.Parameter(torch.empty(cp, cv))
        for p in (self.wa, self.wl, self.wg):
            nn.init.kaiming_uniform_(p, a=5 ** 0.5)


class GDKVM(nn.Module):
    def __init__(self, cfg: Optional[GDKVMConfig] = None):
        super().__init__()
        self.cfg = cfg = cfg or GDKVMConfig()
        if cfg.rule not in _RULES:
            raise ValueError(f"unknown rule {cfg.rule!r}")
        Hh, Dk, Dv, Cp = cfg.heads, cfg.key_dim, cfg.value_dim, cfg.pixel_dim
        if cfg.widths[2] != Cp:
            raise ValueError("pixel_dim must equal the stride-16 encoder width")
        if cfg.normalizer and (cfg.mask_feedback or cfg.scan_segments != 1):
            raise ValueError("normalizer=True runs on the serial scan only (no mask_feedback, scan_segments=1)")
        if cfg.normalizer and not 0.0 < cfg.normalizer_eps < 1.0:
            raise ValueError("normalizer_eps must lie in (0, 1)")
        self.encoder = Encoder(cfg.in_channels, cfg.widths)
        self.key_proj = nn.Conv2d(Cp, Hh * Dk, 1)
        self.query_proj = nn.Conv2d(Cp, Hh * Dk, 1)
        self.value_proj = nn.Conv2d(Cp, Hh * Dv, 1)
        self.mask_embed = nn.Conv2d(1, Hh * Dv, 1, bias=False)
        self.gate_proj = nn.Conv2d(Cp, Hh, 1)
        self.decay_proj = nn.Linear(Cp, Hh)
        nn.init.constant_(self.decay_proj.bias, 2.0)
        self.kpff = KPFFParams(Hh * Dk, Hh * Dv, Cp)
        self.decoder = Decoder(Cp, cfg.widths, cfg.num_classes)
        _Packs().adopt(self)

    def invalidate_packed_weights(self):
        packs = self.__dict__.get("_packs")
        if packs is not None:
            packs.drop_all()
        ops.drop_train_packs(self.__dict__.pop("_train_pack_weights", None) or ())

    def _apply(self, fn, recurse=True):
        self.invalidate_packed_weights()
        return super()._apply(fn, recurse)

    def train(self, mode: bool = True):
        if mode != self.training:
            self.invalidate_packed_weights()
# ... 673 lines not shown
```

gdkvm_amd/ops.py:

```python
from __future__ import annotations

import ctypes
import os
from typing import Optional, Tuple

import torch

RULE_GATED_LINEAR, RULE_DELTA_PARALLEL, RULE_DELTA_SEQUENTIAL = 0, 1, 2
FLAG_NORMALIZE_QK, FLAG_GATE_LOGITS, FLAG_TRAIN, FLAG_WIDE_RANGE = 1, 2, 4, 8


def recurrence_flags(rule: int, flags: int) -> int:
    return flags | FLAG_WIDE_RANGE if rule == RULE_DELTA_PARALLEL else flags
F32, BF16 = 0, 1

_PKG = os.path.dirname(os.path.abspath(__file__))
_SO = os.path.join(_PKG, "libgdkvm_hip.so")
_lib = None
_vp, _sz, _i = ctypes.c_void_p, ctypes.c_size_t, ctypes.c_int

SIGNATURES = {
    "gdkvm_abi_version": (_i, []),
    "gdkvm_last_error": (ctypes.c_char_p, []),
    "gdkvm_scan_workspace_bytes": (_sz, [_i] * 6),
    "gdkvm_scan_fwd": (_i, [_vp] * 10 + [_sz] + [_i] * 9 + [_vp]),
    "gdkvm_scan_prep": (_i, [_vp] * 5 + [_sz] + [_i] * 9 + [_vp]),
    "gdkvm_scan_apply": (_i, [_vp] * 7 + [_sz] + [_i] * 8 + [_vp]),
    "gdkvm_scan_prep_normed": (_i, [_vp] * 6 + [_sz] + [_i] * 9 + [_vp]),
    "gdkvm_scan_fwd_normed": (_i, [_vp] * 10 + [_sz] + [_i] * 9 + [_vp]),
    "gdkvm_scan_transition": (_i, [_vp] * 4 + [_sz] + [_i] * 8 + [_vp]),
    "gdkvm_scan_stitch": (_i, [_vp] * 5 + [_i] * 5 + [_vp]),
    "gdkvm_scan_status": (_i, [_vp, _sz] + [_i] * 7 + [_vp]),
    "gdkvm_scan_bwd_workspace_bytes": (_sz, [_i] * 6),
    "gdkvm_scan_state_bwd": (_i, [_vp] * 6 + [_sz] + [_vp] * 8 + [_sz] + [_i] * 9 + [_vp]),
    "gdkvm_scan_bwd": (_i, [_vp] * 7 + [_sz] + [_vp] * 9 + [_sz] + [_i] * 9 + [_vp]),
    "gdkvm_scan_segments": (_i, [_i] * 5),
    "gdkvm_scan_segmented_workspace_bytes": (_sz, [_i] * 7),
    "gdkvm_scan_fwd_segmented": (_i, [_vp] * 9 + [_sz] + [_i] * 10 + [_vp]),
    "gdkvm_scan_normalizer_workspace_bytes": (_sz, [_i] * 7),
    "gdkvm_scan_fwd_normalizer": (_i, [_vp] * 11 + [_sz] + [_i] * 9 + [ctypes.c_float, _vp]),
    "gdkvm_lkva_read": (_i, [_vp] * 4 + [_i] * 7 + [_vp]),
    "gdkvm_mask_embed_add": (_i, [_vp] * 3 + [_i] * 7 + [_vp]),
    "gdkvm_mask_embed_wgrad_workspace_bytes": (_sz, [_i] * 4),
    "gdkvm_mask_embed_wgrad": (_i, [_vp] * 4 + [_sz] + [_i] * 7 + [_vp]),
    "gdkvm_scan_train_workspace_bytes": (_sz, [_i] * 7),
    "gdkvm_scan_train_fwd": (_i, [_vp] * 9 + [_sz] + [_i] * 9 + [_vp]),
    "gdkvm_scan_train_bwd": (_i, [_vp] * 14 + [_sz] + [_i] * 9 + [_vp]),
    "gdkvm_readout_fwd": (_i, [_vp] * 3 + [_i] * 9 + [_vp]),
    "gdkvm_readout_bwd": (_i, [_vp] * 5 + [_i] * 9 + [_vp]),
    "gdkvm_gemm_nt": (_i, [_vp] * 4 + [_i] * 4 + [_vp]),
    "gdkvm_gemm_tn_workspace_bytes": (_sz, [_i] * 3),
    "gdkvm_gemm_tn": (_i, [_vp] * 4 + [_sz] + [_i] * 4 + [_vp]),
    "gdkvm_gemm_tn_colsum_workspace_bytes": (_sz, [_i] * 3),
    "gdkvm_gemm_tn_colsum": (_i, [_vp] * 5 + [_sz] + [_i] * 4 + [_vp]),
    "gdkvm_kpff_workspace_bytes": (_sz, [_i] * 4),
    "gdkvm_kpff_fwd": (_i, [_vp] * 9 + [_sz] + [_i] * 7 + [_vp]),
    "gdkvm_kpff_fwd_packed": (_i, [_vp] * 9 + [_sz] + [_i] * 7 + [_vp]),
    "gdkvm_kpff_fwd_train": (_i, [_vp] * 13 + [_sz] + [_i] * 7 + [_vp]),
    "gdkvm_kpff_bwd_pre": (_i, [_vp] * 7 + [_i] * 4 + [_vp]),
    "gdkvm_kpff_bwd_post": (_i, [_vp] * 7 + [_i] * 7 + [_vp]),
    "gdkvm_argmax_dice": (_i, [_vp] * 4 + [_i] * 5 + [_vp]),
    "gdkvm_bias_act": (_i, [_vp] * 4 + [_sz] + [_i] * 3 + [_vp]),
    "gdkvm_head_logits": (_i, [_vp] * 4 + [_i] * 6 + [_vp]),
    "gdkvm_head_bwd_workspace_bytes": (_sz, [_i] * 2),
    "gdkvm_head_bwd": (_i, [_vp] * 7 + [_sz] + [_i] * 6 + [_vp]),
    "gdkvm_proj_rows": (_i, [_vp] * 6 + [ctypes.c_longlong] + [_i] * 5 + [_vp]),
    "gdkvm_stem_conv_pool": (_i, [_vp] * 4 + [_i] * 4 + [_vp]),
    "gdkvm_stem_conv_pool_nchw": (_i, [_vp] * 4 + [_i] * 5 + [_vp]),
    "gdkvm_stem_conv_nchw": (_i, [_vp] * 3 + [_i] * 5 + [_vp]),
    "gdkvm_stem_pack_s2d": (_i, [_vp, _vp, _i] + [ctypes.c_longlong] * 4 + [_vp]),
    "gdkvm_stem_wgrad_workspace_bytes": (_sz, [_i] * 3),
    "gdkvm_stem_wgrad_nchw": (_i, [_vp] * 3 + [ctypes.c_longlong] * 4 + [_vp, _sz] + [_i] * 5 + [_vp]),
    "gdkvm_gate_logits": (_i, [_vp] * 7 + [_i] * 5 + [_vp]),
    "gdkvm_proj_gates": (_i, [_vp] * 13 + [_i] * 7 + [_vp]),
    "gdkvm_conv_bias_act": (_i, [_vp] * 5 + [_i] * 12 + [_vp]),
    "gdkvm_conv3x3_pack_weights": (_i, [_vp, _vp, _i, _i, _i, _vp]),
    "gdkvm_conv_igemm_pack_weights": (_i, [_vp, _vp, _i, _i, _i, _i, _i, _vp]),
    "gdkvm_conv_down_bias_act": (_i, [_vp] * 4 + [_i] + [_vp] * 3 + [_i] * 10 + [_vp]),
    "gdkvm_conv_cat_bias_act": (_i, [_vp] * 6 + [_i] * 9 + [_vp]),
    "gdkvm_conv_s2_dgrad_pack_bytes": (_sz, [_i] * 3),
    "gdkvm_conv_s2_pack_train": (_i, [_vp] * 7 + [_i, _i, _vp]),
    "gdkvm_conv_s2_dgrad": (_i, [_vp] * 4 + [_i] * 7 + [_vp]),
    "gdkvm_conv_wgrad_strided_workspace_bytes": (_sz, [_i] * 9),
    "gdkvm_conv_wgrad_strided": (_i, [_vp] * 3 + [ctypes.c_longlong] * 4 + [_vp, _sz] + [_i] * 10 + [_vp]),
    "gdkvm_conv3x3_pack_weights_dgrad": (_i, [_vp, _vp, _i, _i, _i, _vp]),
    "gdkvm_conv3x3_pack_weights_train": (_i, [_i, _vp, _vp, _vp, _vp, _vp, _vp, _vp]),
    "gdkvm_conv3x3_wgrad_workspace_bytes": (_sz, [_i] * 5),
    "gdkvm_conv3x3_wgrad": (_i, [_vp, _vp, _vp, _vp, _sz] + [_i] * 6 + [_vp]),
    "gdkvm_conv3x3_wgrad_krsc": (_i, [_vp, _vp, _vp, _vp, _sz] + [_i] * 6 + [_vp]),
    "gdkvm_upsample_cat": (_i, [_vp] * 3 + [_i] * 8 + [_vp]),
    "gdkvm_upsample_cat_bwd": (_i, [_vp] * 3 + [_i] * 8 + [_vp]),
    "gdkvm_bias_relu_maxpool": (_i, [_vp] * 3 + [_i] * 7 + [_vp]),
    "gdkvm_stem_s2d": (_i, [_vp] * 2 + [_i] * 6 + [_vp]),
    "gdkvm_upsample_argmax_dice": (_i, [_vp] * 4 + [_i] * 7 + [_vp]),
    "gdkvm_head_upsample_argmax_dice": (_i, [_vp] * 6 + [_i] * 8 + [_vp]),
    "gdkvm_maxpool_fwd": (_i, [_vp] * 3 + [_i] * 5 + [_vp]),
    "gdkvm_maxpool_bwd": (_i, [_vp] * 3 + [_i] * 5 + [_vp]),
    "gdkvm_seg_loss_workspace_bytes": (_sz, [_i]),
    "gdkvm_seg_loss_fwd": (_i, [_vp] * 4 + [_sz] + [_i] * 6 + [ctypes.c_float] * 2 + [_i, _i, _vp]),
    "gdkvm_seg_loss_bwd": (_i, [_vp] * 3 + [_sz] + [_vp] * 2 + [_i] * 8 + [_vp]),
    "gdkvm_bn_workspace_bytes": (_sz, [_i]),
    "gdkvm_bn_fwd_train": (_i, [_vp] * 9 + [_sz, ctypes.c_longlong, _i, ctypes.c_float, ctypes.c_float, _i, _i, _vp]),
    "gdkvm_bn_bwd": (_i, [_vp] * 10 + [_sz, ctypes.c_longlong, _i, _i, _i, _vp]),
    "gdkvm_bn_pool_fwd_train": (_i, [_vp] * 9 + [_sz] + [_i] * 4 + [ctypes.c_float] * 2 + [_i, _vp]),
    "gdkvm_bn_pool_bwd": (_i, [_vp] * 9 + [_sz] + [_i] * 5 + [_vp]),
}


class GdkvmError(RuntimeError):
    pass


def library_path() -> str:
    return _SO


def load():
    global _lib
    if _lib is None:
        if not os.path.exists(_SO):
            raise GdkvmError(f"{_SO} not found: build it with `python -m gdkvm_amd.build` "
                             "(there is no fallback path)")
        lib = ctypes.CDLL(_SO)
        for name, (res, args) in SIGNATURES.items():
            fn = getattr(lib, name)
            fn.restype, fn.argtypes = res, args
        if lib.gdkvm_abi_version() != 1:
            raise GdkvmError(f"ABI version mismatch: {lib.gdkvm_abi_version()}")
        _lib = lib
    return _lib


def require_native():
    load()
    if not torch.cuda.is_available():
        raise GdkvmError("no HIP device visible: the GDKVM ops have no CPU path")


def _check(rc: int, what: str):
    if rc != 0:
        raise GdkvmError(f"{what} failed ({rc}): {load().gdkvm_last_error().decode()}")


def _io_dtype(t: torch.Tensor) -> int:
    if t.dtype == torch.float32:
        return F32
    if t.dtype == torch.bfloat16:
        return BF16
    raise GdkvmError(f"unsupported io dtype {t.dtype} (float32 or bfloat16)")


def _dev(*ts):
    dev = None
    for t in ts:
        if t is None:
            continue
        if not t.is_cuda:
            raise GdkvmError("GDKVM ops need device tensors (no CPU path)")
        if not t.is_contiguous():
            raise GdkvmError("GDKVM ops need contiguous tensors")
        if dev is None:
            dev = t.device
        elif t.device != dev:
            raise GdkvmError("tensors on different devices")
    return dev


def _ptr(t: Optional[torch.Tensor]):
    return None if t is None or t.numel() == 0 else t.data_ptr()


def _stream(dev) -> int:
    return torch.cuda.current_stream(dev).cuda_stream


KERNEL_DK = 64


def _pad_keys(q, k, state):
    pad = KERNEL_DK - q.shape[-1]
    Fn = torch.nn.functional
    return Fn.pad(q, (0, pad)), Fn.pad(k, (0, pad)), (None if state is None else Fn.pad(state, (0, 0, 0, pad)))


def scan_workspace_bytes(B, T, Hh, N, Dk, Dv) -> int:
    return int(load().gdkvm_scan_workspace_bytes(B, T, Hh, N, Dk, Dv))


def scan_fwd(q: torch.Tensor, k: torch.Tensor, v: torch.Tensor, alpha: torch.Tensor, beta: torch.Tensor,
             state: Optional[torch.Tensor] = None, rule: int = RULE_DELTA_SEQUENTIAL, flags: int = 0,
             workspace: Optional[torch.Tensor] = None, out: Optional[torch.Tensor] = None,
             state_out: Optional[torch.Tensor] = None, state_hist: Optional[torch.Tensor] = None,
             readout: bool = True, norms: Optional[torch.Tensor] = None, check: bool = False) -> Tuple[Optional[torch.Tensor], torch.Tensor]:
    lib = load()
    if q.dim() != 5 or k.shape != q.shape or v.dim() != 5 or v.shape[:4] != q.shape[:4]:
        raise GdkvmError(f"bad shapes q{tuple(q.shape)} k{tuple(k.shape)} v{tuple(v.shape)}")
    if q.shape[-1] < KERNEL_DK and state_hist is None and q.shape[-1] % 8:
        qp, kp, sp = _pad_keys(q, k, state)
        r, s = scan_fwd(qp, kp, v, alpha, beta, sp, rule, flags, workspace, out, None, None, readout, None, check)
        s = s[:, :, :q.shape[-1]].contiguous()
        if state_out is not None:
            state_out.copy_(s)
            s = state_out
        return r, s
    B, T, N, Hh, Dk = q.shape
    Dv = v.shape[-1]
    if tuple(alpha.shape) != (B, T, Hh) or tuple(beta.shape) != (B, T, N, Hh):
        raise GdkvmError(f"bad gate shapes alpha{tuple(alpha.shape)} beta{tuple(beta.shape)}")
    if k.dtype != q.dtype or v.dtype != q.dtype:
        raise GdkvmError("q, k, v must share one dtype")
    if alpha.dtype != torch.float32 or beta.dtype != torch.float32:
        raise GdkvmError("alpha / beta must be float32")
    if state is not None and (tuple(state.shape) != (B, Hh, Dk, Dv) or state.dtype != torch.float32):
        raise GdkvmError("state must be float32 [B,Hh,Dk,Dv]")
    dev = _dev(q, k, v, alpha, beta, state, workspace, out, state_out, state_hist)
    io = _io_dtype(q)
    need = scan_workspace_bytes(B, T, Hh, N, Dk, Dv)
    if workspace is None:
        workspace = torch.empty(need, dtype=torch.uint8, device=dev)
    r = None if not readout else (out if out is not None else torch.empty((B, T, N, Hh, Dv), dtype=q.dtype, device=dev))
    s = state_out if state_out is not None else torch.empty((B, Hh, Dk, Dv), dtype=torch.float32, device=dev)
    if norms is not None:
        if state_hist is not None or norms.dtype != torch.float32 or norms.numel() != B * T * N * Hh * 2 or not norms.is_contiguous() \
                or norms.device != dev:
            raise GdkvmError("scan_fwd: norms must be contiguous float32 [B*T*N, Hh, 2] on the inputs' device (inference: no state_hist)")
        with torch.cuda.device(dev):
            rc = lib.gdkvm_scan_fwd_normed(_ptr(q), _ptr(k), _ptr(v), _ptr(alpha), _ptr(beta), norms.data_ptr(), _ptr(state), _ptr(r), _ptr(s),
                                           workspace.data_ptr(), workspace.numel() * workspace.element_size(),
                                           B, T, Hh, N, Dk, Dv, io, rule, flags, _stream(dev))
        _check(rc, "gdkvm_scan_fwd_normed")
        if check:
            scan_status(workspace, B, T, Hh, N, Dk, Dv, flags | (FLAG_WIDE_RANGE if rule == RULE_DELTA_PARALLEL else 0))
# ... 965 lines not shown
        _check(rc, "gdkvm_conv_down_bias_act")
        ctx.save_for_backward(xb, dg, weight, down_weight)
        ctx.xdtype = x.dtype
        return y, yd

    @staticmethod
    def backward(ctx, dy, dyd):
        lib = load()
        xb, dg, weight, down_weight = ctx.saved_tensors
        n, c, hh, ww = xb.shape
        k = weight.shape[0]
        cl = torch.channels_last
        dyb = dy.to(torch.bfloat16).contiguous(memory_format=cl)
        dydb = dyd.to(torch.bfloat16).contiguous(memory_format=cl)
        dx = dw = dwd = None
        if ctx.needs_input_grad[0]:
            dx = torch.empty_like(xb)
            with torch.cuda.device(xb.device):
                rc = lib.gdkvm_conv_s2_dgrad(dyb.data_ptr(), dydb.data_ptr(), dg.data_ptr(), dx.data_ptr(), n, c, hh, ww, k, 1, BF16, _stream(xb.device))
            _check(rc, "gdkvm_conv_s2_dgrad")
            dx = dx.to(ctx.xdtype)
        if ctx.needs_input_grad[1]:
            dw = conv_wgrad_strided(xb, dyb, weight, 2, 1).to(weight.dtype)
        if ctx.needs_input_grad[2]:
            dwd = conv_wgrad_strided(xb, dydb, down_weight, 2, 0).to(down_weight.dtype)
        return dx, dw, dwd


def conv_s2_block_served(x: torch.Tensor, conv, down) -> bool:
    w = conv.weight
    k, c = w.shape[:2]
    return (x.is_cuda and x.dim() == 4 and conv.bias is None and down.bias is None and tuple(w.shape[2:]) == (3, 3)
            and tuple(conv.stride) == (2, 2) and tuple(conv.padding) == (1, 1) and tuple(conv.dilation) == (1, 1) and conv.groups == 1
            and conv.padding_mode == "zeros" and tuple(down.weight.shape) == (k, c, 1, 1) and tuple(down.stride) == (2, 2)
            and tuple(down.padding) == (0, 0) and down.groups == 1 and c % 64 == 0 and k % 128 == 0
            and w.dtype == torch.float32 and down.weight.dtype == torch.float32
            and (x.dtype == torch.bfloat16 or (torch.is_autocast_enabled() and torch.get_autocast_dtype("cuda") == torch.bfloat16)))


def conv_s2_block(x: torch.Tensor, weight: torch.Tensor, down_weight: torch.Tensor) -> Tuple[torch.Tensor, torch.Tensor]:
    return _ConvS2BlockFunction.apply(x, weight, down_weight)


def conv_bias_act(x: torch.Tensor, weight: torch.Tensor, bias: torch.Tensor, residual: Optional[torch.Tensor] = None,
                  stride: int = 1, padding: int = 1, relu: bool = True, tile: int = 0,
                  packed: Optional[torch.Tensor] = None) -> torch.Tensor:
    lib = load()
    if x.dim() != 4 or not x.is_cuda or x.dtype != torch.bfloat16 or not x.is_contiguous(memory_format=torch.channels_last):
        raise GdkvmError("conv_bias_act needs a channels_last bf16 [N,C,H,W] device tensor (no CPU path)")
    if weight.dim() != 4 or weight.dtype != torch.bfloat16 or weight.shape[1] != x.shape[1] or \
            not weight.is_contiguous(memory_format=torch.channels_last):
        raise GdkvmError("conv_bias_act: weight must be channels_last bf16 [K,C,R,S]")
    n, c, hh, ww = x.shape
    k, _, r, s = weight.shape
    if bias.dtype != torch.float32 or bias.numel() != k:
        raise GdkvmError("bias must be float32 [K]")
    ho, wo = (hh + 2 * padding - r) // stride + 1, (ww + 2 * padding - s) // stride + 1
    y = torch.empty((n, k, ho, wo), dtype=x.dtype, device=x.device, memory_format=torch.channels_last)
    if residual is not None and (residual.shape != y.shape or residual.dtype != y.dtype or
                                 not residual.is_contiguous(memory_format=torch.channels_last)):
        raise GdkvmError("residual must match the output (shape, dtype, channels_last)")
    with torch.cuda.device(x.device):
        if packed is not None:
            if packed.dtype != torch.bfloat16 or packed.numel() != weight.numel() or packed.device != x.device:
                raise GdkvmError("conv_bias_act: packed must be conv3x3_pack_weights(weight)")
            tile |= CONV_PACKED_WEIGHTS
        rc = lib.gdkvm_conv_bias_act(x.data_ptr(), (packed if packed is not None else weight).data_ptr(), bias.data_ptr(), _ptr(residual),
                                     y.data_ptr(), n, c, hh, ww, k, r, s, stride, padding, int(relu), tile, BF16, _stream(x.device))
    _check(rc, "gdkvm_conv_bias_act")
    return y


def bias_relu_maxpool(x: torch.Tensor, bias: torch.Tensor) -> torch.Tensor:
    lib = load()
    if x.dim() != 4 or not x.is_cuda:
        raise GdkvmError("bias_relu_maxpool needs a channels_last [N,C,H,W] device tensor (or a spatial crop of one)")
    n, c, hh, ww = x.shape
    if x.is_contiguous(memory_format=torch.channels_last):
        x_rows, x_cols = hh, ww
    else:
        sn, sc, sh, sw = x.stride()
        if sc != 1 or sw != c or sh % c or (n > 1 and sn % sh):
            raise GdkvmError("bias_relu_maxpool needs a channels_last [N,C,H,W] device tensor (or a spatial crop of one)")
        x_cols = sh // c
        x_rows = sn // sh if n > 1 else hh
    if bias.dtype != torch.float32 or bias.numel() != c:
        raise GdkvmError("bias must be float32 [C]")
    out = torch.empty((n, c, (hh - 1) // 2 + 1, (ww - 1) // 2 + 1), device=x.device, dtype=x.dtype,
                      memory_format=torch.channels_last)
    with torch.cuda.device(x.device):
        rc = lib.gdkvm_bias_relu_maxpool(x.data_ptr(), bias.data_ptr(), out.data_ptr(), n, hh, ww, c, x_rows, x_cols,
                                         _io_dtype(x), _stream(x.device))
    _check(rc, "gdkvm_bias_relu_maxpool")
    return out


def stem_s2d(x: torch.Tensor, cpad: int) -> torch.Tensor:
    lib = load()
    if x.dim() != 4 or not x.is_cuda or not x.is_contiguous():
        raise GdkvmError("stem_s2d needs a contiguous NCHW device tensor")
    n, c, hh, ww = x.shape
    out = torch.empty((n, cpad, hh // 2, ww // 2), device=x.device, dtype=x.dtype, memory_format=torch.channels_last)
    with torch.cuda.device(x.device):
        rc = lib.gdkvm_stem_s2d(x.data_ptr(), out.data_ptr(), n, c, hh, ww, cpad, _io_dtype(x), _stream(x.device))
    _check(rc, "gdkvm_stem_s2d")
    return out


def upsample_bilinear(lo: torch.Tensor, size) -> torch.Tensor:
    lib = load()
    if lo.dim() != 4 or not lo.is_cuda or lo.dtype != torch.bfloat16 or not lo.is_contiguous(memory_format=torch.channels_last):
        raise GdkvmError("upsample_bilinear needs a channels_last bf16 [N,C,h,w] device tensor (no CPU path)")
    n, c1, hl, wl = lo.shape
    H, W = int(size[0]), int(size[1])
    out = torch.empty((n, c1, H, W), dtype=lo.dtype, device=lo.device, memory_format=torch.channels_last)
    with torch.cuda.device(lo.device):
        rc = lib.gdkvm_upsample_cat(lo.data_ptr(), None, out.data_ptr(), n, hl, wl, H, W, c1, 0, BF16, _stream(lo.device))
    _check(rc, "gdkvm_upsample_cat")
    return out


def conv_cat_bias_act(x1: torch.Tensor, x2: torch.Tensor, weight: torch.Tensor, bias: torch.Tensor,
                      residual: Optional[torch.Tensor] = None, relu: bool = True, tile: int = 0,
                      packed: Optional[torch.Tensor] = None) -> torch.Tensor:
    lib = load()
    for t in (x1, x2):
        if t.dim() != 4 or not t.is_cuda or t.dtype != torch.bfloat16 or not t.is_contiguous(memory_format=torch.channels_last):
            raise GdkvmError("conv_cat_bias_act needs channels_last bf16 [N,C,H,W] device tensors (no CPU path)")
    n, c1, hh, ww = x1.shape
    c2 = x2.shape[1]
    if tuple(x2.shape) != (n, c2, hh, ww):
        raise GdkvmError("conv_cat_bias_act: x1 and x2 must agree in batch and size")
    if weight.dim() != 4 or weight.dtype != torch.bfloat16 or tuple(weight.shape[1:]) != (c1 + c2, 3, 3) or \
            not weight.is_contiguous(memory_format=torch.channels_last):
        raise GdkvmError("conv_cat_bias_act: weight must be channels_last bf16 [K,C1+C2,3,3]")
    k = weight.shape[0]
    if bias.dtype != torch.float32 or bias.numel() != k:
        raise GdkvmError("bias must be float32 [K]")
    y = torch.empty((n, k, hh, ww), dtype=x1.dtype, device=x1.device, memory_format=torch.channels_last)
    if residual is not None and (residual.shape != y.shape or residual.dtype != y.dtype or
                                 not residual.is_contiguous(memory_format=torch.channels_last)):
        raise GdkvmError("residual must match the output (shape, dtype, channels_last)")
    if packed is not None:
        if packed.dtype != torch.bfloat16 or packed.numel() != weight.numel() or packed.device != x1.device:
            raise GdkvmError("conv_cat_bias_act: packed must be conv3x3_pack_weights(weight)")
        tile |= CONV_PACKED_WEIGHTS
    with torch.cuda.device(x1.device):
        rc = lib.gdkvm_conv_cat_bias_act(x1.data_ptr(), x2.data_ptr(), (packed if packed is not None else weight).data_ptr(), bias.data_ptr(),
                                         _ptr(residual), y.data_ptr(), n, c1, c2, hh, ww, k, int(relu), tile, BF16, _stream(x1.device))
    _check(rc, "gdkvm_conv_cat_bias_act")
    return y


def _upsample_cat_fwd(lo: torch.Tensor, skip: torch.Tensor) -> torch.Tensor:
    lib = load()
    for t in (lo, skip):
        if t.dim() != 4 or not t.is_cuda or not t.is_contiguous(memory_format=torch.channels_last):
            raise GdkvmError("upsample_cat needs channels_last device tensors")
    if lo.dtype != torch.bfloat16 or skip.dtype != torch.bfloat16 or lo.shape[0] != skip.shape[0]:
        raise GdkvmError("upsample_cat: bf16 tensors with equal batch")
    n, c1, hl, wl = lo.shape
    _, c2, H, W = skip.shape
    out = torch.empty((n, c1 + c2, H, W), dtype=lo.dtype, device=lo.device, memory_format=torch.channels_last)
    with torch.cuda.device(lo.device):
        rc = lib.gdkvm_upsample_cat(lo.data_ptr(), skip.data_ptr(), out.data_ptr(), n, hl, wl, H, W, c1, c2, BF16, _stream(lo.device))
    _check(rc, "gdkvm_upsample_cat")
    return out


def stem_conv_pool(xs: torch.Tensor, w_s2d: torch.Tensor, bias: torch.Tensor) -> torch.Tensor:
    lib = load()
    if xs.dim() != 4 or not xs.is_cuda or xs.dtype != torch.bfloat16 or xs.shape[1] != 16 or \
            not xs.is_contiguous(memory_format=torch.channels_last):
        raise GdkvmError("stem_conv_pool needs a channels_last bf16 [N,16,Hs,Ws] device tensor (no CPU path)")
    if tuple(w_s2d.shape) != (64, 16, 4, 4) or w_s2d.dtype != torch.bfloat16 or not w_s2d.is_contiguous(memory_format=torch.channels_last):
        raise GdkvmError("stem_conv_pool: weight must be channels_last bf16 [64,16,4,4]")
    if bias.dtype != torch.float32 or bias.numel() != 64:
        raise GdkvmError("bias must be float32 [64]")
    n, _, hs, ws = xs.shape
    y = torch.empty((n, 64, (hs - 1) // 2 + 1, (ws - 1) // 2 + 1), dtype=xs.dtype, device=xs.device, memory_format=torch.channels_last)
    with torch.cuda.device(xs.device):
        rc = lib.gdkvm_stem_conv_pool(xs.data_ptr(), w_s2d.data_ptr(), bias.data_ptr(), y.data_ptr(), n, hs, ws, BF16, _stream(xs.device))
    _check(rc, "gdkvm_stem_conv_pool")
    return y


def stem_conv_pool_nchw(x: torch.Tensor, w_s2d: torch.Tensor, bias: torch.Tensor) -> torch.Tensor:
    lib = load()
    if x.dim() != 4 or not x.is_cuda or x.dtype != torch.bfloat16 or not x.is_contiguous() or x.shape[1] > 4 or x.shape[2] % 2 or x.shape[3] % 2:
        raise GdkvmError("stem_conv_pool_nchw needs a contiguous NCHW bf16 [N, C <= 4, H, W] device tensor with even H, W (no CPU path)")
    if tuple(w_s2d.shape) != (64, 16, 4, 4) or w_s2d.dtype != torch.bfloat16 or not w_s2d.is_contiguous(memory_format=torch.channels_last):
        raise GdkvmError("stem_conv_pool: weight must be channels_last bf16 [64,16,4,4]")
    if bias.dtype != torch.float32 or bias.numel() != 64:
        raise GdkvmError("bias must be float32 [64]")
    n, c, hh, ww = x.shape
    hs, ws = hh // 2, ww // 2
    y = torch.empty((n, 64, (hs - 1) // 2 + 1, (ws - 1) // 2 + 1), dtype=x.dtype, device=x.device, memory_format=torch.channels_last)
    with torch.cuda.device(x.device):
        rc = lib.gdkvm_stem_conv_pool_nchw(x.data_ptr(), w_s2d.data_ptr(), bias.data_ptr(), y.data_ptr(), n, c, hh, ww, BF16, _stream(x.device))
    _check(rc, "gdkvm_stem_conv_pool_nchw")
    return y


class _StemConvFunction(torch.autograd.Function):

    @staticmethod
    def forward(ctx, x, weight):
        lib = load()
        xb = x.detach().to(torch.bfloat16).contiguous()
        n, c, hh, ww = xb.shape
        w4 = torch.empty(64 * 256, dtype=torch.bfloat16, device=xb.device)
        y = torch.empty((n, 64, hh // 2, ww // 2), dtype=torch.bfloat16, device=xb.device, memory_format=torch.channels_last)
        wd = weight.detach()
        with torch.cuda.device(xb.device):
            _check(lib.gdkvm_stem_pack_s2d(wd.data_ptr(), w4.data_ptr(), c, *wd.stride(), _stream(xb.device)), "gdkvm_stem_pack_s2d")
            _check(lib.gdkvm_stem_conv_nchw(xb.data_ptr(), w4.data_ptr(), y.data_ptr(), n, c, hh, ww, BF16, _stream(xb.device)), "gdkvm_stem_conv_nchw")
        ctx.save_for_backward(xb, weight)
        return y

    @staticmethod
    def backward(ctx, dy):
        xb, weight = ctx.saved_tensors
        dw = None
        if ctx.needs_input_grad[1]:
            dw = stem_wgrad(xb, dy, like=weight)
        return None, dw


def stem_wgrad(x: torch.Tensor, dy: torch.Tensor, like: Optional[torch.Tensor] = None) -> torch.Tensor:
    lib = load()
    xb = x.detach().to(torch.bfloat16).contiguous()
    dyb = _nhwc(dy.detach(), "stem_wgrad")
    if dyb.dtype != torch.bfloat16:
        dyb = dyb.to(torch.bfloat16)
    n, c, hh, ww = xb.shape
    if tuple(dyb.shape) != (n, 64, hh // 2, ww // 2):
        raise GdkvmError(f"stem_wgrad: dy {tuple(dyb.shape)} does not match x {tuple(xb.shape)}")
    dw = torch.empty_like(like, dtype=torch.float32) if like is not None else torch.empty((64, c, 7, 7), dtype=torch.float32, device=xb.device)
    need = lib.gdkvm_stem_wgrad_workspace_bytes(n, hh, ww)
    ws = torch.empty(need, dtype=torch.uint8, device=xb.device)
    with torch.cuda.device(xb.device):
        _check(lib.gdkvm_stem_wgrad_nchw(xb.data_ptr(), dyb.data_ptr(), dw.data_ptr(), *dw.stride(), ws.data_ptr(), need, n, c, hh, ww, BF16,
                                         _stream(xb.device)), "gdkvm_stem_wgrad_nchw")
    return dw


def stem_conv_served(x: torch.Tensor, conv) -> bool:
    w = conv.weight
    return (x.is_cuda and x.dim() == 4 and x.shape[1] <= 4 and x.shape[2] % 2 == 0 and x.shape[3] % 2 == 0 and conv.bias is None
            and tuple(w.shape) == (64, x.shape[1], 7, 7) and w.dtype == torch.float32 and conv.stride == (2, 2) and conv.padding == (3, 3)
            and conv.dilation == (1, 1) and conv.groups == 1 and conv.padding_mode == "zeros"
            and (x.dtype == torch.bfloat16 or (torch.is_autocast_enabled() and torch.get_autocast_dtype("cuda") == torch.bfloat16)))


def stem_conv(x: torch.Tensor, weight: torch.Tensor) -> torch.Tensor:
    return _StemConvFunction.apply(x, weight)


def upsample_cat_bwd(dout: torch.Tensor, lo_shape, skip_shape) -> Tuple[torch.Tensor, torch.Tensor]:
    lib = load()
    dout = _nhwc(dout, "upsample_cat_bwd")
    if dout.dtype != torch.bfloat16:
        dout = dout.to(torch.bfloat16)
    n, c1, hl, wl = lo_shape
    _, c2, H, W = skip_shape
    if tuple(dout.shape) != (n, c1 + c2, H, W):
        raise GdkvmError(f"upsample_cat_bwd: d_out {tuple(dout.shape)} does not match {lo_shape} + {skip_shape}")
    dlo = torch.empty((n, c1, hl, wl), dtype=dout.dtype, device=dout.device, memory_format=torch.channels_last)
    dskip = torch.empty((n, c2, H, W), dtype=dout.dtype, device=dout.device, memory_format=torch.channels_last)
    with torch.cuda.device(dout.device):
        rc = lib.gdkvm_upsample_cat_bwd(dout.data_ptr(), dlo.data_ptr(), dskip.data_ptr(), n, hl, wl, H, W, c1, c2, BF16,
                                        _stream(dout.device))
    _check(rc, "gdkvm_upsample_cat_bwd")
    return dlo, dskip


class _UpsampleCatFunction(torch.autograd.Function):
    @staticmethod
    def forward(ctx, lo, skip):
        ctx.shapes = (tuple(lo.shape), tuple(skip.shape))
        return _upsample_cat_fwd(lo, skip)

    @staticmethod
    def backward(ctx, dout):
        return upsample_cat_bwd(dout, *ctx.shapes)


def upsample_cat(lo: torch.Tensor, skip: torch.Tensor) -> torch.Tensor:
    if torch.is_grad_enabled() and (lo.requires_grad or skip.requires_grad):
        return _UpsampleCatFunction.apply(lo, skip)
    return _upsample_cat_fwd(lo, skip)


def _nhwc(t: torch.Tensor, what: str) -> torch.Tensor:
    if t.dim() != 4 or not t.is_cuda:
        raise GdkvmError(f"{what}: needs a [N,C,H,W] device tensor (no CPU path)")
    return t.contiguous(memory_format=torch.channels_last)


def bn_act_fwd(x, weight, bias, running_mean=None, running_var=None, residual=None, momentum: float = 0.1, eps: float = 1e-5,
               relu: bool = True):
    lib = load()
    x = _nhwc(x, "bn_act_fwd")
    n, c, hh, ww = x.shape
    if residual is not None:
        residual = _nhwc(residual, "bn_act_fwd")
# ... 326 lines not shown
```

include/gdkvm.h:

```cpp
#ifndef GDKVM_H
#define GDKVM_H

#include <stddef.h>
#include <stdint.h>

#ifdef __cplusplus
extern "C" {
#endif

#define GDKVM_ABI_VERSION 1

enum { GDKVM_OK = 0, GDKVM_ERR_SHAPE = -1, GDKVM_ERR_DTYPE = -2, GDKVM_ERR_ARCH = -3,
       GDKVM_ERR_LAUNCH = -4, GDKVM_ERR_WORKSPACE = -5, GDKVM_ERR_ARG = -6,
       GDKVM_ERR_RANGE = -7  };

enum { GDKVM_F32 = 0, GDKVM_BF16 = 1 };

enum { GDKVM_RULE_GATED_LINEAR = 0,
       GDKVM_RULE_DELTA_PARALLEL = 1,
       GDKVM_RULE_DELTA_SEQUENTIAL = 2    };

enum { GDKVM_FLAG_NORMALIZE_QK = 1,
       GDKVM_FLAG_GATE_LOGITS = 2,
       GDKVM_FLAG_TRAIN = 4,
// ... 18 lines not shown
                     int B, int T, int Hh, int N, int Dk, int Dv, int io_dtype, int flags, void* stream);

int gdkvm_scan_prep_normed(const void* q, const void* k, const void* v, const float* beta, const float* norms,
                           void* workspace, size_t workspace_bytes,
                           int B, int T, int Hh, int N, int Dk, int Dv, int io_dtype, int rule, int flags, void* stream);
int gdkvm_scan_fwd_normed(const void* q, const void* k, const void* v, const float* alpha, const float* beta, const float* norms,
                          const float* s_in, void* r_out, float* s_out, void* workspace, size_t workspace_bytes,
                          int B, int T, int Hh, int N, int Dk, int Dv, int io_dtype, int rule, int flags, void* stream);

int gdkvm_scan_transition(const void* q, const float* alpha, float* phi_out, const void* workspace, size_t workspace_bytes,
                          int B, int T, int Hh, int N, int Dk, int Dv, int io_dtype, int flags, void* stream);
int gdkvm_scan_stitch(const float* phi, const float* s_loc, const float* s_in, float* starts, float* s_end,
                      int B, int S, int Hh, int Dk, int Dv, void* stream);

int gdkvm_scan_segments(int B, int T, int Hh, int Dv, int segments);
size_t gdkvm_scan_segmented_workspace_bytes(int B, int T, int Hh, int N, int Dk, int Dv, int segments);
int gdkvm_scan_fwd_segmented(const void* q, const void* k, const void* v, const float* alpha, const float* beta,
                             const float* s_in, void* r_out, float* s_out, void* workspace, size_t workspace_bytes,
                             int B, int T, int Hh, int N, int Dk, int Dv, int segments,
                             int io_dtype, int rule, int flags, void* stream);

size_t gdkvm_scan_normalizer_workspace_bytes(int B, int T, int Hh, int N, int Dk, int Dv, int io_dtype);
int gdkvm_scan_fwd_normalizer(const void* q, const void* k, const void* v, const float* alpha, const float* beta,
                              const float* s_in, const float* z_in, void* r_out, float* s_out, float* z_out,
                              void* workspace, size_t workspace_bytes,
                              int B, int T, int Hh, int N, int Dk, int Dv, int io_dtype, int rule, int flags, float eps, void* stream);

int gdkvm_lkva_read(const void* q, const float* norms, const float* s, void* r_out,
                    int B, int N, int Hh, int Dk, int Dv, int io_dtype, int flags, void* stream);
int gdkvm_mask_embed_add(const uint8_t* mask, const float* w_embed, void* v, int BT, int H, int W, int h, int w, int C,
                         int io_dtype, void* stream);
size_t gdkvm_mask_embed_wgrad_workspace_bytes(int F, int h, int w, int C);
int gdkvm_mask_embed_wgrad(const uint8_t* mask, const void* d_v, float* d_w, void* workspace, size_t workspace_bytes,
                           int F, int H, int W, int h, int w, int C, int io_dtype, void* stream);

size_t gdkvm_scan_bwd_workspace_bytes(int B, int T, int Hh, int N, int Dk, int Dv);
int gdkvm_scan_bwd(const void* q, const void* k, const void* v, const float* alpha, const float* beta,
                   const float* s_hist, const void* fwd_workspace, size_t fwd_workspace_bytes,
                   const void* d_r, const float* d_s_out,
                   void* d_q, void* d_k, void* d_v, float* d_alpha, float* d_beta, float* d_s_in,
                   void* bwd_workspace, size_t bwd_workspace_bytes,
                   int B, int T, int Hh, int N, int Dk, int Dv, int io_dtype, int rule, int flags, void* stream);

size_t gdkvm_scan_train_workspace_bytes(int B, int T, int Hh, int N, int Dk, int Dv, int io_dtype);
int gdkvm_scan_train_fwd(const void* q, const void* k, const void* v, const float* alpha, const float* beta, const float* s_in,
                         void* r_out, float* s_out, void* train_workspace, size_t train_workspace_bytes,
                         int B, int T, int Hh, int N, int Dk, int Dv, int io_dtype, int rule, int flags, void* stream);
int gdkvm_scan_train_bwd(const void* q, const void* k, const void* v, const float* alpha, const float* beta,
                         const void* d_r, const float* d_s_out,
                         void* d_q, void* d_k, void* d_v, float* d_alpha, float* d_beta, float* d_s_in,
                         void* train_workspace, size_t train_workspace_bytes,
                         int B, int T, int Hh, int N, int Dk, int Dv, int io_dtype, int rule, int flags, void* stream);

int gdkvm_scan_state_bwd(const void* k, const void* v, const float* alpha, const float* beta,
                         const float* s_hist, const void* fwd_workspace, size_t fwd_workspace_bytes,
                         const float* d_hist, const float* d_s_out,
                         void* d_k, void* d_v, float* d_alpha, float* d_beta, float* d_s_in,
                         void* bwd_workspace, size_t bwd_workspace_bytes,
                         int B, int T, int Hh, int N, int Dk, int Dv, int io_dtype, int rule, int flags, void* stream);

int gdkvm_readout_fwd(const void* q, const float* s_hist, void* r_out, int B, int T, int Hh, int N, int Dk, int Dv,
                      int hist_stride, int io_dtype, int flags, void* stream);
int gdkvm_readout_bwd(const void* q, const float* s_hist, const void* d_r, void* d_q, float* d_hist,
                      int B, int T, int Hh, int N, int Dk, int Dv, int hist_stride, int io_dtype, int flags, void* stream);

int gdkvm_gemm_nt(const void* a, const void* b, const float* bias, void* c, int M, int N, int K, int io_dtype, void* stream);
size_t gdkvm_gemm_tn_workspace_bytes(int M, int K1, int N);
int gdkvm_gemm_tn(const void* a, const void* b, float* c, void* workspace, size_t workspace_bytes,
                  int M, int K1, int N, int io_dtype, void* stream);
size_t gdkvm_gemm_tn_colsum_workspace_bytes(int M, int K1, int N);
int gdkvm_gemm_tn_colsum(const void* a, const void* b, float* c, float* colsum, void* workspace, size_t workspace_bytes,
                         int M, int K1, int N, int io_dtype, void* stream);

size_t gdkvm_kpff_workspace_bytes(int Ck, int Cv, int Cp, int io_dtype);
int gdkvm_kpff_fwd(const void* local, const void* global, const void* pixel,
                   const float* wa, const float* ba, const float* wl, const float* wg, void* out,
                   void* workspace, size_t workspace_bytes,
                   int BT, int Ck, int Cv, int Cp, int h, int w, int io_dtype, void* stream);

int gdkvm_kpff_fwd_packed(const void* local, const void* global, const void* pixel,
                          const float* wa, const float* ba, const float* wl, const float* wg, void* out,
                          void* packed_workspace, size_t workspace_bytes,
                          int BT, int Ck, int Cv, int Cp, int h, int w, int io_dtype, void* stream);

int gdkvm_kpff_fwd_train(const void* local, const void* global, const void* pixel,
                         const float* wa, const float* ba, const float* wl, const float* wg, void* out,
                         void* save_gates, void* save_lp, void* save_gp, void* save_gms,
                         void* workspace, size_t workspace_bytes,
                         int BT, int Ck, int Cv, int Cp, int h, int w, int io_dtype, void* stream);
int gdkvm_kpff_bwd_pre(const void* d_out, const void* gates, const void* lp, const void* gp,
                       void* d_z, void* d_lp, void* d_gp, int BT, int N, int Cp, int io_dtype, void* stream);
int gdkvm_kpff_bwd_post(const void* d_out, const void* d_x, const void* d_l_add, const void* d_g_add,
                        void* d_pixel, void* d_local, void* d_global,
                        int BT, int Ck, int Cv, int Cp, int h, int w, int io_dtype, void* stream);

int gdkvm_argmax_dice(const void* logits, const uint8_t* target, uint8_t* mask, int32_t* counts,
                      int BT, int ncls, int H, int W, int io_dtype, void* stream);

int gdkvm_upsample_argmax_dice(const void* logits, const uint8_t* target, uint8_t* mask, int32_t* counts,
                               int BT, int ncls, int hl, int wl, int H, int W, int io_dtype, void* stream);

int gdkvm_head_upsample_argmax_dice(const void* x, const float* w, const float* b, const uint8_t* target, uint8_t* mask,
                                    int32_t* counts, int BT, int C, int ncls, int hl, int wl, int H, int W, int io_dtype, void* stream);

int gdkvm_bias_act(const void* x, const float* bias, const void* residual, void* y,
                   size_t rows, int C, int relu, int io_dtype, void* stream);

int gdkvm_head_logits(const void* x, const float* w, const float* b, void* out, int N, int H, int W, int C, int classes,
                      int io_dtype, void* stream);
size_t gdkvm_head_bwd_workspace_bytes(int C, int ncls);
int gdkvm_head_bwd(const void* x, const void* dz, const float* w, void* dx, float* dw, float* db, void* workspace, size_t workspace_bytes,
                   int N, int H, int W, int C, int ncls, int io_dtype, void* stream);

int gdkvm_proj_rows(const void* x, const void* wpack, const float* bias, void* out0, void* out1, void* out2,
                    long long rows, int K, int w0, int w1, int w2, int io_dtype, void* stream);

int gdkvm_gate_logits(const void* p, const float* w_gate, const float* b_gate, const float* w_decay, const float* b_decay,
                      float* beta, float* alpha, int frames, int N, int Cp, int Hh, int io_dtype, void* stream);

int gdkvm_proj_gates(const void* x, const void* wpack, const float* bias, void* out_k, void* out_q, void* out_v,
                     const float* w_gate, const float* b_gate, const float* w_decay, const float* b_decay,
                     float* beta, float* alpha, float* norms,
                     int frames, int N, int K, int Hh, int Dk, int Dv, int io_dtype, void* stream);

enum { GDKVM_CONV_PACKED_WEIGHTS = 32 };
int gdkvm_conv3x3_pack_weights(const void* w, void* packed, int K, int C, int io_dtype, void* stream);
int gdkvm_conv_igemm_pack_weights(const void* w, void* packed, int K, int C, int R, int S, int io_dtype, void* stream);
int gdkvm_conv3x3_pack_weights_dgrad(const void* w, void* packed, int K, int C, int io_dtype, void* stream);
#define GDKVM_PACK_MAX_LAYERS 24
int gdkvm_conv3x3_pack_weights_train(int nlayers, const void* const* w, void* const* packed_fwd, void* const* packed_dgrad,
                                     const int* K, const int* C, const long long* strides, void* stream);
size_t gdkvm_conv3x3_wgrad_workspace_bytes(int N, int C, int H, int W, int K);
int gdkvm_conv3x3_wgrad(const void* x, const void* dy, float* dw, void* workspace, size_t workspace_bytes,
                        int N, int C, int H, int W, int K, int io_dtype, void* stream);
int gdkvm_conv3x3_wgrad_krsc(const void* x, const void* dy, float* dw, void* workspace, size_t workspace_bytes,
                        int N, int C, int H, int W, int K, int io_dtype, void* stream);
int gdkvm_conv_bias_act(const void* x, const void* w, const float* bias, const void* residual, void* y,
                        int N, int C, int H, int W, int K, int R, int S, int stride, int pad, int relu, int kernel,
                        int io_dtype, void* stream);
int gdkvm_conv_down_bias_act(const void* x, const void* w, const float* bias, void* y, int relu,
                             const void* w_down, const float* bias_down, void* y_down,
                             int N, int C, int H, int W, int K, int R, int S, int stride, int pad, int io_dtype, void* stream);
size_t gdkvm_conv_s2_dgrad_pack_bytes(int C, int K, int with_down);
int gdkvm_conv_s2_pack_train(const float* w, const long long* w_strides, const float* w_down, const long long* w_down_strides,
                             void* packed_fwd, void* packed_fwd_down, void* packed_dgrad, int K, int C, void* stream);
int gdkvm_conv_s2_dgrad(const void* dy, const void* dy_down, const void* packed_dgrad, void* dx,
                        int N, int C, int H, int W, int K, int with_down, int io_dtype, void* stream);
size_t gdkvm_conv_wgrad_strided_workspace_bytes(int N, int C, int H, int W, int K, int R, int S, int stride, int pad);
int gdkvm_conv_wgrad_strided(const void* x, const void* dy, float* dw, long long sk, long long sc, long long sr, long long ss,
                             void* workspace, size_t workspace_bytes,
                             int N, int C, int H, int W, int K, int R, int S, int stride, int pad, int io_dtype, void* stream);
int gdkvm_conv_cat_bias_act(const void* x1, const void* x2, const void* w, const float* bias, const void* residual, void* y,
                            int N, int C1, int C2, int H, int W, int K, int relu, int kernel, int io_dtype, void* stream);

int gdkvm_bias_relu_maxpool(const void* x, const float* bias, void* y, int N, int H, int W, int C,
                            int x_rows, int x_cols, int io_dtype, void* stream);

int gdkvm_stem_conv_pool(const void* xs, const void* w, const float* bias, void* y, int N, int Hs, int Ws,
                         int io_dtype, void* stream);
int gdkvm_stem_conv_pool_nchw(const void* x, const void* w, const float* bias, void* y, int N, int C, int H, int W,
                              int io_dtype, void* stream);
int gdkvm_stem_conv_nchw(const void* x, const void* w4, void* y, int N, int C, int H, int W, int io_dtype, void* stream);
int gdkvm_stem_pack_s2d(const float* w7, void* w4, int C, long long sk, long long sc, long long sr, long long ss, void* stream);
size_t gdkvm_stem_wgrad_workspace_bytes(int N, int H, int W);
int gdkvm_stem_wgrad_nchw(const void* x, const void* dy, float* dw, long long sk, long long sc, long long sr, long long ss,
                          void* workspace, size_t workspace_bytes, int N, int C, int H, int W, int io_dtype, void* stream);

int gdkvm_maxpool_fwd(const void* x, void* y, void* idx, int N, int H, int W, int C, int io_dtype, void* stream);
int gdkvm_maxpool_bwd(const void* dy, const void* idx, void* dx, int N, int H, int W, int C, int io_dtype, void* stream);

int gdkvm_stem_s2d(const void* x, void* out, int N, int C, int H, int W, int Cp, int io_dtype, void* stream);

size_t gdkvm_bn_workspace_bytes(int C);
int gdkvm_bn_fwd_train(const void* x, const void* residual, const float* gamma, const float* beta,
                       float* running_mean, float* running_var, void* y, float* save_stats,
                       void* ws, size_t ws_bytes, long long rows, int C, float eps, float momentum, int relu,
                       int io_dtype, void* stream);
int gdkvm_bn_bwd(const void* x, const void* y, const void* dy, const float* gamma, const float* save_stats,
                 void* dx, void* dres, float* dgamma, float* dbeta, void* ws, size_t ws_bytes,
                 long long rows, int C, int relu, int io_dtype, void* stream);
int gdkvm_bn_pool_fwd_train(const void* x, const float* gamma, const float* beta, float* running_mean, float* running_var,
                            void* y_pool, void* idx, float* save_stats, void* ws, size_t ws_bytes,
                            int N, int H, int W, int C, float eps, float momentum, int io_dtype, void* stream);
int gdkvm_bn_pool_bwd(const void* x, const void* dy_pool, const void* idx, const float* gamma, const float* save_stats,
                      void* dx, float* dgamma, float* dbeta, void* ws, size_t ws_bytes,
                      int N, int H, int W, int C, int io_dtype, void* stream);

int gdkvm_upsample_cat(const void* lo, const void* skip, void* out,
                       int Nimg, int hl, int wl, int H, int W, int C1, int C2, int io_dtype, void* stream);
int gdkvm_upsample_cat_bwd(const void* dout, void* dlo, void* dskip,
                           int Nimg, int hl, int wl, int H, int W, int C1, int C2, int io_dtype, void* stream);

size_t gdkvm_seg_loss_workspace_bytes(int C);
int gdkvm_seg_loss_fwd(const void* z, const void* target, float* out, void* ws, size_t ws_bytes,
                       int images, int C, int h, int w, int H, int W, float dice_weight, float eps,
                       int io_dtype, int target_bytes, void* stream);
int gdkvm_seg_loss_bwd(const void* z, const void* target, const void* ws, size_t ws_bytes, const float* grad_out, void* dz,
                       int images, int C, int h, int w, int H, int W, int io_dtype, int target_bytes, void* stream);

#ifdef __cplusplus
}
#endif
#endif
```

Measured before the change: 631,600 frames/s.

## Fuse 2x bilinear upsample into concat 3x3 conv tile kernel

Adds an UP variant of the tiled 3x3 conv kernel. It stages the low-resolution decoder input into LDS and expands it bilinearly 2x in LDS before the MMA loop, so the separate upsample kernel and its full-resolution intermediate tensor are no longer needed. The decoder block takes this fused path by default when the shapes qualify. In exchange it adds an extra LDS staging area and extra barriers plus expansion work inside each chunk iteration, which can lower occupancy and delay the pipeline. It also changes the lerp arithmetic to explicit FMA with fp contraction turned off.

Result: no change. 636,600 frames/s (median of 6 runs) (+0.8%).

```diff
diff --git a/gdkvm_amd/csrc/conv3x3_tile.hip b/gdkvm_amd/csrc/conv3x3_tile.hip
--- a/gdkvm_amd/csrc/conv3x3_tile.hip
+++ b/gdkvm_amd/csrc/conv3x3_tile.hip
@@ -10,6 +10,7 @@
 constexpr int CT_SLOTS = CT_PIX / 16;
 constexpr int CT_MAXMT = 13;
 constexpr int CT_VARIANT_128 = 4, CT_VARIANT_64 = 3;
+constexpr int CT_UP_PIECES = 12;
 
 __device__ const uint4 g_ct_zero16 = {0, 0, 0, 0};
 
@@ -20,6 +21,12 @@
         f(std::integral_constant<int, I>{});
         static_for_ct<I + 1, E>(f);
     }
+}
+
+__device__ __forceinline__ unsigned ct_pack_bf16x2(gdkvm_f32x2 v)
+{
+    typedef __bf16 bf16x2 __attribute__((ext_vector_type(2)));
+    return __builtin_bit_cast(unsigned, __builtin_convertvector(v, bf16x2));
 }
 
 struct ConvTileArgs {
@@ -31,6 +38,8 @@
     int relu;
     float inv_band, inv_bw, inv_tw, inv_w;
     int perm;
+    int hl, wl, srows, spieces;
+    float inv_sband, inv_wl, inv_nrp, inv_ncp;
 };
 
 __device__ __forceinline__ int ct_div(int n, float inv) { return (int)(((float)n + 0.5f) * inv); }
@@ -40,9 +49,10 @@
     return perm ? 32 * (kt >> 1) + 8 * (j >> 2) + 4 * (kt & 1) + (j & 3) : 16 * kt + j;
 }
 
-template <int NWN, int NTW, bool PK, int NWV = 8, int MAXMT = CT_MAXMT>
+template <int NWN, int NTW, bool PK, int NWV = 8, int MAXMT = CT_MAXMT, bool UP = false>
 __global__ __launch_bounds__(64 * NWV, (NWV == 4 ? 2 : 1)) void conv3x3_tile_kernel(ConvTileArgs a)
 {
+    static_assert(!UP || NWV == 4, "the enlarged-input form exists for the four-wave grids");
     constexpr int MW = NWV / NWN, MTW = (MAXMT + MW - 1) / MW;
     extern __shared__ __attribute__((aligned(16))) unsigned char ct_band[];
     const int tid = threadIdx.x, lane = tid & 63, li = lane & 15, g = lane >> 4;
@@ -70,6 +80,7 @@
         const bool live = j < a.npieces && c < 8 && pix < a.band_px && bx >= 1 && bx <= W;
         g_meta[u] = live ? (by << 16 | (c * 8) << 8 | f) : -1;
     }
+    constexpr int SPU = UP ? CT_UP_PIECES / NWV : 0;
     struct Geo { const bf16_t* b1; const bf16_t* b2; int y0, nfr; };
     auto geo_of = [&](int tile) __attribute__((always_inline)) {
         const int ty = tile % a.tiles_y, fg = tile / a.tiles_y;
@@ -77,7 +88,8 @@
         q.y0 = ty * a.th - 1;
         q.nfr = min(a.fpt, a.N - fg * a.fpt);
         const long long px0 = ((long long)fg * a.fpt * H + q.y0) * W - 1;
-        q.b1 = a.x + px0 * (a.x2 ? a.C1 : C);
+        if constexpr (UP) q.b1 = a.x + ((long long)fg * a.fpt * a.hl + ((q.y0 - 1) >> 1)) * a.wl * a.C1;
+        else q.b1 = a.x + px0 * (a.x2 ? a.C1 : C);
         q.b2 = a.x2 ? a.x2 + px0 * (C - a.C1) - a.C1 : a.x;
         return q;
     };
@@ -86,15 +98,35 @@
         const bool second = a.x2 != nullptr && chunk * CT_CK >= a.C1;
         const int cs = a.x2 ? (second ? C - a.C1 : a.C1) : C;
         const bf16_t* origin = (second ? q.b2 : q.b1) + chunk * CT_CK;
-#pragma unroll
-        for (int u = 0; u < PP; ++u) {
+        const bool low = UP && !second;
+        static_for_ct<0, PP>([&](auto uc) {
+            constexpr int u = decltype(uc)::value;
             const int j = w + NWV * u;
-            const int yy = y0 + (g_meta[u] >> 16);
-            const bool ok = g_meta[u] >= 0 && (unsigned)yy < (unsigned)H && (g_meta[u] & 255) < nfr;
-            const bf16_t* src = ok ? origin + g_pix[u] * cs + ((g_meta[u] >> 8) & 255) : reinterpret_cast<const bf16_t*>(&g_ct_zero16);
-            unsigned char* dst = j < a.npieces ? ct_band + buf * band_bytes + 1024 * j : ct_band + 2 * band_bytes;
+            const bf16_t* src;
+            unsigned char* dst;
+            if constexpr (!UP) {
+                const int yy = y0 + (g_meta[u] >> 16);
+                const bool ok = g_meta[u] >= 0 && (unsigned)yy < (unsigned)H && (g_meta[u] & 255) < nfr;
+                src = ok ? origin + g_pix[u] * cs + ((g_meta[u] >> 8) & 255) : reinterpret_cast<const bf16_t*>(&g_ct_zero16);
+                dst = j < a.npieces ? ct_band + buf * band_bytes + 1024 * j : ct_band + 2 * band_bytes;
+            } else {
+                int meta = g_meta[u], pixo = g_pix[u];
+                if (low) {
+                    meta = -1; pixo = 0;
+                    if constexpr (u < SPU) {
+                        const int e = 64 * j + lane, pix = e >> 3;
+                        const int f = ct_div(pix, a.inv_sband), r = pix - f * (a.srows * a.wl), sy = ct_div(r, a.inv_wl), sx = r - sy * a.wl;
+                        pixo = (f * a.hl + sy) * a.wl + sx;
+                        if (j < a.spieces && pix < a.fpt * a.srows * a.wl) meta = sy << 16 | ((e & 7) * 8) << 8 | f;
+                    }
+                }
+                const int yy = (low ? (y0 - 1) >> 1 : y0) + (meta >> 16);
+                const bool ok = meta >= 0 && (unsigned)yy < (unsigned)(low ? a.hl : H) && (meta & 255) < nfr;
+                src = ok ? origin + pixo * cs + ((meta >> 8) & 255) : reinterpret_cast<const bf16_t*>(&g_ct_zero16);
+                dst = j < (low ? a.spieces : a.npieces) ? (low ? ct_band + 2 * band_bytes + 1024 : ct_band + buf * band_bytes) + 1024 * j : ct_band + 2 * band_bytes;
+            }
             __builtin_amdgcn_global_load_lds(src, reinterpret_cast<__attribute__((address_space(3))) void*>(reinterpret_cast<uintptr_t>(dst)), 16, 0, 0);
-        }
+        });
     };
 
     int tile = blockIdx.x;
@@ -135,11 +167,64 @@
         if constexpr (NTW == 1) asm volatile("s_waitcnt vmcnt(%1)" : "+v"(o.f[0]) : "n"(N) : "memory");
         else asm volatile("s_waitcnt vmcnt(%2)" : "+v"(o.f[0]), "+v"(o.f[1]) : "n"(N) : "memory");
     };
+    auto ct_expand = [&](int y0, int nfr, int buf) __attribute__((always_inline)) {
+        const int s0 = (y0 - 1) >> 1;
+        unsigned char* const band = ct_band + buf * band_bytes;
+        unsigned char* const dump = ct_band + 2 * band_bytes + lane * 16;
+        const unsigned char* const stage = dump - lane * 16 + 1024;
+        const int nrp = a.srows - 1, ncp = a.wl + 1, nblk = a.fpt * nrp * ncp * 8;
+        for (int i = tid; i < nblk; i += 64 * NWV) {
+            const int bi = i >> 3, c = i & 7;
+            const int t = ct_div(bi, a.inv_ncp), cp = bi - t * ncp, f = ct_div(t, a.inv_nrp), rp = t - f * nrp;
+            const int ip = s0 + rp, jp = cp - 1;
+            const int r0 = min(max(max(ip, 0) - s0, 0), nrp), r1 = min(max(min(ip + 1, a.hl - 1) - s0, 0), nrp);
+            const int x0 = max(jp, 0), x1 = min(jp + 1, a.wl - 1);
+            const unsigned char* const s0p = stage + ((f * a.srows + r0) * a.wl) * 128 + c * 16;
+            const unsigned char* const s1p = stage + ((f * a.srows + r1) * a.wl) * 128 + c * 16;
+            const uint4 t00 = *reinterpret_cast<const uint4*>(s0p + x0 * 128), t01 = *reinterpret_cast<const uint4*>(s0p + x1 * 128);
+            const uint4 t10 = *reinterpret_cast<const uint4*>(s1p + x0 * 128), t11 = *reinterpret_cast<const uint4*>(s1p + x1 * 128);
+            const unsigned ta[4] = {t00.x, t00.y, t00.z, t00.w}, tb[4] = {t01.x, t01.y, t01.z, t01.w};
+            const unsigned tc[4] = {t10.x, t10.y, t10.z, t10.w}, td[4] = {t11.x, t11.y, t11.z, t11.w};
+            const int yy = 2 * ip + 1, by = yy - y0;
+            const float ly1 = yy + 1 <= 0 ? 0.f : 0.75f, hy1 = 1.f - ly1;
+            unsigned o[2][2][4];
+#pragma unroll
+            for (int q = 0; q < 4; ++q) {
+                const gdkvm_f32x2 pa = {__uint_as_float(ta[q] << 16), __uint_as_float(ta[q] & 0xffff0000u)}, pb = {__uint_as_float(tb[q] << 16), __uint_as_float(tb[q] & 0xffff0000u)};
+                const gdkvm_f32x2 pc = {__uint_as_float(tc[q] << 16), __uint_as_float(tc[q] & 0xffff0000u)}, pd = {__uint_as_float(td[q] << 16), __uint_as_float(td[q] & 0xffff0000u)};
+#pragma unroll
+                for (int e = 0; e < 2; ++e) {
+                    const float lx = e ? 0.75f : 0.25f, hx = 1.f - lx;
+                    const gdkvm_f32x2 u0 = gdkvm_lerp(pa, pb, hx, lx), u1 = gdkvm_lerp(pc, pd, hx, lx);
+                    const gdkvm_f32x2 v0 = gdkvm_lerp(u0, u1, 0.75f, 0.25f), v1 = gdkvm_lerp(u0, u1, hy1, ly1);
+                    o[0][e][q] = ct_pack_bf16x2(v0);
+                    o[1][e][q] = ct_pack_bf16x2(v1);
+                }
+            }
+#pragma unroll
+            for (int ey = 0; ey < 2; ++ey) {
+                const bool inband = (unsigned)(by + ey) < (unsigned)a.bh;
+                const bool rowok = f < nfr && (unsigned)(yy + ey) < (unsigned)H;
+                unsigned char* const row = band + ((f * a.bh + by + ey) * BW + 2 * cp) * CT_PIX + c * 16;
+#pragma unroll
+                for (int e = 0; e < 2; ++e) {
+                    const bool ok = rowok && (unsigned)(2 * jp + 1 + e) < (unsigned)W;
+                    *reinterpret_cast<uint4*>(inband ? row + e * CT_PIX : dump) =
+                        ok ? make_uint4(o[ey][e][0], o[ey][e][1], o[ey][e][2], o[ey][e][3]) : make_uint4(0u, 0u, 0u, 0u);
+                }
+            }
+        }
+    };
     int gc = 0;
     constexpr int WD = 3, KU = 6;
     WF wr[WD];
 #pragma unroll
     for (int j = 0; j < WD; ++j) wload(wr[j], j);
+    if constexpr (UP) {
+        asm volatile("s_waitcnt vmcnt(%0)" ::"n"(WD * NTW) : "memory");
+        asm volatile("s_barrier" ::: "memory");
+        ct_expand(cur.y0, cur.nfr, 0);
+    }
     for (; tile < a.ntiles; tile += gridDim.x) {
         const Geo nxt = geo_of(min(tile + (int)gridDim.x, a.ntiles - 1));
         f32x4 acc[MTW][NTW];
@@ -192,6 +277,14 @@
             trip(0, std::true_type{});
 #pragma unroll 1
             for (int r0 = KU; r0 < 18; r0 += KU) trip(r0, std::false_type{});
+            if constexpr (UP) {
+                const bool more = chunk + 1 < nchunk;
+                if ((more ? chunk + 1 : 0) * CT_CK < a.C1 && (more || tile + (int)gridDim.x < a.ntiles)) {
+                    asm volatile("s_waitcnt vmcnt(%0)" ::"n"(WD * NTW) : "memory");
+                    asm volatile("s_barrier" ::: "memory");
+                    ct_expand(more ? cur.y0 : nxt.y0, more ? cur.nfr : nxt.nfr, buf ^ 1);
+                }
+            }
         }
         {
             const int ty = tile % a.tiles_y, fg = tile / a.tiles_y;
@@ -199,7 +292,7 @@
             auto pk4 = [](const f32x4& v) { return make_uint2((unsigned)f32_to_bf16(v[0]) | ((unsigned)f32_to_bf16(v[1]) << 16), (unsigned)f32_to_bf16(v[2]) | ((unsigned)f32_to_bf16(v[3]) << 16)); };
             const float lo = a.relu ? 0.f : -INFINITY;
             typedef float f32x2 __attribute__((ext_vector_type(2)));
-            if (NTW == 2 && a.perm) {
+            if (NTW == 2 && (UP || a.perm)) {
                 if (co0 < K) {
                     unsigned o[MTW];
 #pragma unroll
@@ -408,19 +501,30 @@
     return hipFuncSetAttribute(reinterpret_cast<const void*>(conv3x3_tile_kernel<NWN, NTW, true, NWV, MAXMT>), hipFuncAttributeMaxDynamicSharedMemorySize, 113 * 1024) == hipSuccess
         && hipFuncSetAttribute(reinterpret_cast<const void*>(conv3x3_tile_kernel<NWN, NTW, false, NWV, MAXMT>), hipFuncAttributeMaxDynamicSharedMemorySize, 113 * 1024) == hipSuccess;
 }
-}
-
-int gdkvm_conv3x3_tile_launch(const void* x, const void* x2, int C1, const void* w, const float* bias, const void* residual, void* y,
-                              int N, int C, int H, int W, int K, int relu, int variant, int packed, hipStream_t st)
+constexpr size_t CT_UP_LDS = 80 * 1024;
+template <int NWN, int NTW>
+void launch_tile_up(dim3 grid, size_t lds, hipStream_t st, const ConvTileArgs& a)
+{
+    hipLaunchKernelGGL((conv3x3_tile_kernel<NWN, NTW, true, 4, 7, true>), grid, dim3(256), lds, st, a);
+}
+template <int NWN, int NTW>
+bool setattr_tile_up()
+{
+    return hipFuncSetAttribute(reinterpret_cast<const void*>(conv3x3_tile_kernel<NWN, NTW, true, 4, 7, true>), hipFuncAttributeMaxDynamicSharedMemorySize, (int)CT_UP_LDS) == hipSuccess;
+}
+
+int tile_launch(const void* x, const void* x2, int C1, const void* w, const float* bias, const void* residual, void* y,
+                int N, int C, int H, int W, int K, int relu, int variant, int packed, bool up, hipStream_t st)
 {
     if (variant == 0 && K % 128 == 0 && CT_VARIANT_128 == 4) {
-        if (gdkvm_conv3x3_tile_launch(x, x2, C1, w, bias, residual, y, N, C, H, W, K, relu, 4, packed, st) == 0) return 0;
+        if (tile_launch(x, x2, C1, w, bias, residual, y, N, C, H, W, K, relu, 4, packed, up, st) == 0) return 0;
         variant = 2;
     }
     if (variant == 0 && K % 128 != 0 && (H * W <= 16 * 7 || 2 * W <= 16 * 7)) {
-        if (gdkvm_conv3x3_tile_launch(x, x2, C1, w, bias, residual, y, N, C, H, W, K, relu, 5, packed, st) == 0) return 0;
+        if (tile_launch(x, x2, C1, w, bias, residual, y, N, C, H, W, K, relu, 5, packed, up, st) == 0) return 0;
         variant = 3;
     }
+    if (up && ((variant != 4 && variant != 5) || !x2 || !packed || H % 2 || W % 2 || K % 32)) return 1;
     if (C % CT_CK || K % 16 || W > 64 || W < 1 || H < 1 || N < 1 || variant < 0 || variant > 5) return 1;
     if (variant == 4 && K % 128) return 1;
     const bool half = variant == 4 || variant == 5;
@@ -450,7 +554,15 @@
     if (variant == 0) variant = K % 128 == 0 ? 2 : CT_VARIANT_64;
     const int kwg = (variant == 2 || variant == 4) ? 128 : 64;
     const int gy = (K + kwg - 1) / kwg;
-    const size_t lds = (size_t)2 * a.npieces * 1024 + 1024;
+    a.hl = H / 2; a.wl = W / 2; a.srows = a.bh / 2 + 2; a.spieces = 0;
+    if (up) {
+        a.spieces = (a.fpt * a.srows * a.wl * 8 + 63) / 64;
+        if (a.spieces > CT_UP_PIECES) return 1;
+    }
+    a.inv_sband = 1.0f / (float)(a.srows * a.wl); a.inv_wl = 1.0f / (float)a.wl;
+    a.inv_nrp = 1.0f / (float)(a.srows - 1); a.inv_ncp = 1.0f / (float)(a.wl + 1);
+    const size_t lds = (size_t)2 * a.npieces * 1024 + 1024 + (size_t)a.spieces * 1024;
+    if (up && lds > CT_UP_LDS) return 1;
     int per = (half ? 512 : 256) / gy; if (per < 1) per = 1;
     const int gx = (int)(ntiles < per ? ntiles : per);
     static std::atomic<unsigned long long> done_mask{0};
@@ -458,8 +570,14 @@
     if (hipGetDevice(&dev) != hipSuccess) return 1;
     const unsigned long long bit = 1ull << (dev & 63);
     if (!(done_mask.load(std::memory_order_relaxed) & bit)) {
-        if (!setattr_tile<4, 1>() || !setattr_tile<4, 2>() || !setattr_tile<2, 2>() || !setattr_tile<4, 2, 4, 7>() || !setattr_tile<2, 2, 4, 7>()) return 1;
+        if (!setattr_tile<4, 1>() || !setattr_tile<4, 2>() || !setattr_tile<2, 2>() || !setattr_tile<4, 2, 4, 7>() || !setattr_tile<2, 2, 4, 7>()
+            || !setattr_tile_up<4, 2>() || !setattr_tile_up<2, 2>()) return 1;
         done_mask.fetch_or(bit, std::memory_order_relaxed);
+    }
+    if (up) {
+        if (variant == 4) launch_tile_up<4, 2>(dim3(gx, gy), lds, st, a);
+        else launch_tile_up<2, 2>(dim3(gx, gy), lds, st, a);
+        return 0;
     }
     switch (variant) {
         case 1: launch_tile<4, 1>(packed, dim3(gx, gy), lds, st, a); break;
@@ -470,3 +588,17 @@
     }
     return 0;
 }
+}
+
+int gdkvm_conv3x3_tile_launch(const void* x, const void* x2, int C1, const void* w, const float* bias, const void* residual, void* y,
+                              int N, int C, int H, int W, int K, int relu, int variant, int packed, hipStream_t st)
+{
+    return tile_launch(x, x2, C1, w, bias, residual, y, N, C, H, W, K, relu, variant, packed, false, st);
+}
+
+int gdkvm_conv3x3_tile_up2x_launch(const void* x, const void* x2, int C1, const void* w, const float* bias, const void* residual, void* y,
+                                   int N, int C, int H, int W, int K, int relu, int variant, int packed, hipStream_t st)
+{
+    if (variant != 0 && variant != 4 && variant != 5) return 1;
+    return tile_launch(x, x2, C1, w, bias, residual, y, N, C, H, W, K, relu, variant, packed, true, st);
+}
diff --git a/gdkvm_amd/csrc/conv_dispatch.hip b/gdkvm_amd/csrc/conv_dispatch.hip
--- a/gdkvm_amd/csrc/conv_dispatch.hip
+++ b/gdkvm_amd/csrc/conv_dispatch.hip
@@ -4,6 +4,8 @@
                              int relu, int packed, hipStream_t st);
 int gdkvm_conv3x3_tile_launch(const void* x, const void* x2, int C1, const void* w, const float* bias, const void* residual, void* y,
                               int N, int C, int H, int W, int K, int relu, int variant, int packed, hipStream_t st);
+int gdkvm_conv3x3_tile_up2x_launch(const void* x, const void* x2, int C1, const void* w, const float* bias, const void* residual, void* y,
+                                   int N, int C, int H, int W, int K, int relu, int variant, int packed, hipStream_t st);
 int gdkvm_conv_igemm_launch(const void* x, const void* wpacked, const float* bias, const void* residual, void* y,
                             int N, int C, int H, int W, int K, int R, int S, int stride, int pad, int relu,
                             const void* w2packed, const float* bias2, void* y2, hipStream_t st);
@@ -83,6 +85,30 @@
     return GDKVM_OK;
 }
 
+extern "C" int gdkvm_conv_up2x_cat_bias_act(const void* x1, const void* x2, const void* w, const float* bias, const void* residual, void* y,
+                                            int N, int C1, int C2, int H, int W, int K, int relu, int kernel, int io_dtype, void* stream)
+{
+    if (io_dtype != GDKVM_BF16) return gdkvm_fail(GDKVM_ERR_DTYPE, "conv_up2x_cat_bias_act: only bf16 is implemented");
+    const bool packed = kernel & GDKVM_CONV_PACKED_WEIGHTS;
+    kernel &= ~GDKVM_CONV_PACKED_WEIGHTS;
+    if (kernel != 0 && kernel != 10 && kernel != 11) return gdkvm_fail(GDKVM_ERR_ARG, "conv_up2x_cat_bias_act: kernel=%d (0, 10, 11)", kernel);
+    if (N < 0 || C1 <= 0 || C2 <= 0 || C1 % 64 || C2 % 64 || H <= 0 || W <= 0 || H % 2 || W % 2 || W > 64 || K <= 0 || K % 32)
+        return gdkvm_fail(GDKVM_ERR_SHAPE, "conv_up2x_cat_bias_act: N=%d C1=%d C2=%d H=%d W=%d K=%d is not served (C1, C2 multiples of 64, K of 32, "
+                                           "H and W even, rows of at most 64 pixels)", N, C1, C2, H, W, K);
+    if (!packed) return gdkvm_fail(GDKVM_ERR_SHAPE, "conv_up2x_cat_bias_act: plain weights are not served (gdkvm_conv3x3_pack_weights, flag %d)", GDKVM_CONV_PACKED_WEIGHTS);
+    if (N == 0) return GDKVM_OK;
+    if (!x1 || !x2 || !w || !bias || !y) return gdkvm_fail(GDKVM_ERR_ARG, "conv_up2x_cat_bias_act: null pointer");
+    if (!gdkvm_aligned16(x1) || !gdkvm_aligned16(x2) || !gdkvm_aligned16(w) || !gdkvm_aligned16(y) || !gdkvm_aligned16(bias) || (residual && !gdkvm_aligned16(residual)))
+        return gdkvm_fail(GDKVM_ERR_ARG, "conv_up2x_cat_bias_act: pointers must be 16-byte aligned");
+    if ((size_t)N * H * W * (C1 + C2) >= (1ull << 31) || (size_t)N * H * W * K >= (1ull << 31))
+        return gdkvm_fail(GDKVM_ERR_SHAPE, "conv_up2x_cat_bias_act: tensor too large for 32-bit offsets");
+    if (int rc = gdkvm_check_device()) return rc;
+    if (gdkvm_conv3x3_tile_up2x_launch(x1, x2, C1, w, bias, residual, y, N, C1 + C2, H, W, K, relu, kernel ? kernel - 6 : 0, 1, static_cast<hipStream_t>(stream)))
+        return gdkvm_fail(GDKVM_ERR_SHAPE, "conv_up2x_cat_bias_act: N=%d C1=%d C2=%d %dx%d K=%d is not served by the four-wave tile grids", N, C1, C2, H, W, K);
+    GDKVM_LAUNCH_CHECK("conv3x3_tile_kernel");
+    return GDKVM_OK;
+}
+
 extern "C" int gdkvm_conv_down_bias_act(const void* x, const void* w, const float* bias, void* y, int relu,
                                         const void* w_down, const float* bias_down, void* y_down,
                                         int N, int C, int H, int W, int K, int R, int S, int stride, int pad, int io_dtype, void* stream)
diff --git a/gdkvm_amd/csrc/epilogue.hip b/gdkvm_amd/csrc/epilogue.hip
--- a/gdkvm_amd/csrc/epilogue.hip
+++ b/gdkvm_amd/csrc/epilogue.hip
@@ -247,8 +247,8 @@
                     unsigned r[4];
 #pragma unroll
                     for (int q = 0; q < 4; ++q) {
-                        const float v0 = hy * (hx * a[2 * q] + lx * b[2 * q]) + ly * (hx * cc[2 * q] + lx * d[2 * q]);
-                        const float v1 = hy * (hx * a[2 * q + 1] + lx * b[2 * q + 1]) + ly * (hx * cc[2 * q + 1] + lx * d[2 * q + 1]);
+                        const float v0 = gdkvm_bilerp(a[2 * q], b[2 * q], cc[2 * q], d[2 * q], hx, lx, hy, ly);
+                        const float v1 = gdkvm_bilerp(a[2 * q + 1], b[2 * q + 1], cc[2 * q + 1], d[2 * q + 1], hx, lx, hy, ly);
                         r[q] = (unsigned)f32_to_bf16(v0) | ((unsigned)f32_to_bf16(v1) << 16);
                     }
                     *reinterpret_cast<uint4*>(orow + x * C + c) = make_uint4(r[0], r[1], r[2], r[3]);
@@ -281,8 +281,8 @@
                 unsigned r[4];
 #pragma unroll
                 for (int q = 0; q < 4; ++q) {
-                    const float v0 = hy * (hx * a[2 * q] + lx[u] * b[2 * q]) + ly * (hx * cc[2 * q] + lx[u] * d[2 * q]);
-                    const float v1 = hy * (hx * a[2 * q + 1] + lx[u] * b[2 * q + 1]) + ly * (hx * cc[2 * q + 1] + lx[u] * d[2 * q + 1]);
+                    const float v0 = gdkvm_bilerp(a[2 * q], b[2 * q], cc[2 * q], d[2 * q], hx, lx[u], hy, ly);
+                    const float v1 = gdkvm_bilerp(a[2 * q + 1], b[2 * q + 1], cc[2 * q + 1], d[2 * q + 1], hx, lx[u], hy, ly);
                     r[q] = (unsigned)f32_to_bf16(v0) | ((unsigned)f32_to_bf16(v1) << 16);
                 }
                 *reinterpret_cast<uint4*>(orow + oidx[u]) = make_uint4(r[0], r[1], r[2], r[3]);
@@ -347,8 +347,8 @@
                     unsigned r[4];
 #pragma unroll
                     for (int q = 0; q < 4; ++q) {
-                        const float v0 = hy * (hx * a[2 * q] + lx * b[2 * q]) + ly * (hx * cc[2 * q] + lx * d[2 * q]);
-                        const float v1 = hy * (hx * a[2 * q + 1] + lx * b[2 * q + 1]) + ly * (hx * cc[2 * q + 1] + lx * d[2 * q + 1]);
+                        const float v0 = gdkvm_bilerp(a[2 * q], b[2 * q], cc[2 * q], d[2 * q], hx, lx, hy, ly);
+                        const float v1 = gdkvm_bilerp(a[2 * q + 1], b[2 * q + 1], cc[2 * q + 1], d[2 * q + 1], hx, lx, hy, ly);
                         r[q] = (unsigned)f32_to_bf16(v0) | ((unsigned)f32_to_bf16(v1) << 16);
                     }
                     *reinterpret_cast<uint4*>(orow + x * C + c) = make_uint4(r[0], r[1], r[2], r[3]);
diff --git a/gdkvm_amd/csrc/gdkvm_common.hpp b/gdkvm_amd/csrc/gdkvm_common.hpp
--- a/gdkvm_amd/csrc/gdkvm_common.hpp
+++ b/gdkvm_amd/csrc/gdkvm_common.hpp
@@ -36,6 +36,22 @@
 }
 __device__ __forceinline__ float sigmoidf_(float x) { return 1.0f / (1.0f + __expf(-x)); }
 
+__device__ __forceinline__ float gdkvm_lerp(float a, float b, float h, float l)
+{
+#pragma clang fp contract(off)
+    return __builtin_fmaf(h, a, l * b);
+}
+typedef float gdkvm_f32x2 __attribute__((ext_vector_type(2)));
+__device__ __forceinline__ gdkvm_f32x2 gdkvm_lerp(gdkvm_f32x2 a, gdkvm_f32x2 b, float h, float l)
+{
+#pragma clang fp contract(off)
+    return __builtin_elementwise_fma(gdkvm_f32x2{h, h}, a, gdkvm_f32x2{l, l} * b);
+}
+__device__ __forceinline__ float gdkvm_bilerp(float a, float b, float c, float d, float hx, float lx, float hy, float ly)
+{
+    return gdkvm_lerp(gdkvm_lerp(a, b, hx, lx), gdkvm_lerp(c, d, hx, lx), hy, ly);
+}
+
 template <int IO>
 __device__ __forceinline__ f32x4 load4(const void* base, size_t off)
 {
diff --git a/gdkvm_amd/model.py b/gdkvm_amd/model.py
--- a/gdkvm_amd/model.py
+++ b/gdkvm_amd/model.py
@@ -257,12 +257,17 @@
         self.conv = nn.Sequential(nn.Conv2d(cin + cskip, cout, 3, 1, 1, bias=False), _bn(cout), nn.ReLU(inplace=True),
                                   nn.Conv2d(cout, cout, 3, 1, 1, bias=False), _bn(cout), nn.ReLU(inplace=True))
 
+    fuse_upsample = True
+
     def forward(self, x, skip):
         c = self.conv
         if (isinstance(c[0], FusedConv) and not torch.is_grad_enabled() and x.is_cuda and x.dtype == torch.bfloat16
                 and skip.dtype == torch.bfloat16 and c[0].cat_served(x.shape[1], skip.shape[1], skip.shape[-1])):
-            u = ops.upsample_bilinear(x.contiguous(memory_format=torch.channels_last), skip.shape[2:])
-            y = c[0].forward_cat(u, skip)
+            if self.fuse_upsample and c[0].up2x_cat_served(x.shape, skip.shape):
+                y = c[0].forward_up2x_cat(x, skip)
+            else:
+                u = ops.upsample_bilinear(x.contiguous(memory_format=torch.channels_last), skip.shape[2:])
+                y = c[0].forward_cat(u, skip)
             for m in list(c)[1:]:
                 y = m(y)
             return y
@@ -367,6 +372,16 @@
                 and cv.dilation == (1, 1) and cv.stride == (1, 1) and cv.padding == (1, 1) and cv.weight.is_cuda
                 and cv.weight.dtype == torch.bfloat16 and cv.weight.is_contiguous(memory_format=torch.channels_last)
                 and c1 % 64 == 0 and c2 % 64 == 0 and c1 + c2 == cv.in_channels and cv.out_channels % 16 == 0 and width <= 64)
+
+    def up2x_cat_served(self, lo_shape, skip_shape) -> bool:
+        (n, c1, hl, wl), (n2, c2, h, w) = lo_shape, skip_shape
+        return (n == n2 and (h, w) == (2 * hl, 2 * wl) and self.cat_served(c1, c2, w)
+                and ops.conv_up2x_served(c1, c2, self.conv.out_channels, h, w))
+
+    def forward_up2x_cat(self, x1, x2):
+        cl = torch.channels_last
+        return ops.conv_up2x_cat_bias_act(x1.contiguous(memory_format=cl), x2.contiguous(memory_format=cl), self.conv.weight, self.epi.bias,
+                                          None, self.relu, 0, self._packed(x1.device))
 
     def forward_cat(self, x1, x2):
         cl = torch.channels_last
diff --git a/gdkvm_amd/ops.py b/gdkvm_amd/ops.py
--- a/gdkvm_amd/ops.py
+++ b/gdkvm_amd/ops.py
@@ -78,6 +78,7 @@
     "gdkvm_conv_igemm_pack_weights": (_i, [_vp, _vp, _i, _i, _i, _i, _i, _vp]),
     "gdkvm_conv_down_bias_act": (_i, [_vp] * 4 + [_i] + [_vp] * 3 + [_i] * 10 + [_vp]),
     "gdkvm_conv_cat_bias_act": (_i, [_vp] * 6 + [_i] * 9 + [_vp]),
+    "gdkvm_conv_up2x_cat_bias_act": (_i, [_vp] * 6 + [_i] * 9 + [_vp]),
     "gdkvm_conv_s2_dgrad_pack_bytes": (_sz, [_i] * 3),
     "gdkvm_conv_s2_pack_train": (_i, [_vp] * 7 + [_i, _i, _vp]),
     "gdkvm_conv_s2_dgrad": (_i, [_vp] * 4 + [_i] * 7 + [_vp]),
@@ -1349,6 +1350,56 @@
     return y
 
 
+def conv_up2x_served(c1: int, c2: int, k: int, h: int, w: int) -> bool:
+    if c1 <= 0 or c2 <= 0 or c1 % 64 or c2 % 64 or k <= 0 or k % 32 or h <= 0 or w <= 0 or h % 2 or w % 2 or w > 64:
+        return False
+    if k % 128 and not (h * w <= 112 or 2 * w <= 112):
+        return False
+    if h * w <= 112:
+        th, fpt = h, 112 // (h * w)
+    else:
+        th, fpt = 112 // w, 1
+    pieces = lambda: (fpt * (th + 2) * (w + 2) * 10 + 63) // 64
+    while pieces() > 32 and fpt > 1:
+        fpt -= 1
+    while pieces() > 32 and th > 1:
+        th -= 1
+    if pieces() > 32:
+        return False
+    staging = (fpt * ((th + 2) // 2 + 2) * (w // 2) * 8 + 63) // 64
+    return staging <= 12 and 2 * pieces() + 1 + staging <= 80
+
+
+def conv_up2x_cat_bias_act(x1: torch.Tensor, x2: torch.Tensor, weight: torch.Tensor, bias: torch.Tensor,
+                           residual: Optional[torch.Tensor] = None, relu: bool = True, tile: int = 0,
+                           packed: Optional[torch.Tensor] = None) -> torch.Tensor:
+    lib = load()
+    for t in (x1, x2):
+        if t.dim() != 4 or not t.is_cuda or t.dtype != torch.bfloat16 or not t.is_contiguous(memory_format=torch.channels_last):
+            raise GdkvmError("conv_up2x_cat_bias_act needs channels_last bf16 [N,C,H,W] device tensors (no CPU path)")
+    n, c1, hl, wl = x1.shape
+    c2, hh, ww = x2.shape[1:]
+    if x2.shape[0] != n or (hh, ww) != (2 * hl, 2 * wl):
+        raise GdkvmError("conv_up2x_cat_bias_act: x2 must have x1's batch and exactly twice its size")
+    if weight.dim() != 4 or weight.dtype != torch.bfloat16 or tuple(weight.shape[1:]) != (c1 + c2, 3, 3) or \
+            not weight.is_contiguous(memory_format=torch.channels_last):
+        raise GdkvmError("conv_up2x_cat_bias_act: weight must be channels_last bf16 [K,C1+C2,3,3]")
+    k = weight.shape[0]
+    if bias.dtype != torch.float32 or bias.numel() != k:
+        raise GdkvmError("bias must be float32 [K]")
+    if packed is None or packed.dtype != torch.bfloat16 or packed.numel() != weight.numel() or packed.device != x1.device:
+        raise GdkvmError("conv_up2x_cat_bias_act: packed must be conv3x3_pack_weights(weight)")
+    y = torch.empty((n, k, hh, ww), dtype=x1.dtype, device=x1.device, memory_format=torch.channels_last)
+    if residual is not None and (residual.shape != y.shape or residual.dtype != y.dtype or
+                                 not residual.is_contiguous(memory_format=torch.channels_last)):
+        raise GdkvmError("residual must match the output (shape, dtype, channels_last)")
+    with torch.cuda.device(x1.device):
+        rc = lib.gdkvm_conv_up2x_cat_bias_act(x1.data_ptr(), x2.data_ptr(), packed.data_ptr(), bias.data_ptr(), _ptr(residual), y.data_ptr(),
+                                              n, c1, c2, hh, ww, k, int(relu), tile | CONV_PACKED_WEIGHTS, BF16, _stream(x1.device))
+    _check(rc, "gdkvm_conv_up2x_cat_bias_act")
+    return y
+
+
 def _upsample_cat_fwd(lo: torch.Tensor, skip: torch.Tensor) -> torch.Tensor:
     lib = load()
     for t in (lo, skip):
diff --git a/include/gdkvm.h b/include/gdkvm.h
--- a/include/gdkvm.h
+++ b/include/gdkvm.h
@@ -194,6 +194,8 @@
                              int N, int C, int H, int W, int K, int R, int S, int stride, int pad, int io_dtype, void* stream);
 int gdkvm_conv_cat_bias_act(const void* x1, const void* x2, const void* w, const float* bias, const void* residual, void* y,
                             int N, int C1, int C2, int H, int W, int K, int relu, int kernel, int io_dtype, void* stream);
+int gdkvm_conv_up2x_cat_bias_act(const void* x1, const void* x2, const void* w, const float* bias, const void* residual, void* y,
+                                 int N, int C1, int C2, int H, int W, int K, int relu, int kernel, int io_dtype, void* stream);
 
 int gdkvm_bias_relu_maxpool(const void* x, const float* bias, void* y, int N, int H, int W, int C,
                             int x_rows, int x_cols, int io_dtype, void* stream);
```
